# google-research/rigl

Measured on NVIDIA H100. Metric: sparse_train_step_images_per_sec_resnet50_erk80, higher is better.
Workload: dtype bf16

## Files before the change

include/rigl_b200.h:

```cpp
#ifndef RIGL_B200_H_
#define RIGL_B200_H_

#include <stddef.h>
#include <stdint.h>

#if defined(__GNUC__)
#define RIGL_API __attribute__((visibility("default")))
#else
#define RIGL_API
#endif

#ifdef __cplusplus
extern "C" {
#endif

typedef enum {
  RIGL_OK = 0,
  RIGL_ERR_INVALID_ARG = -1,
  RIGL_ERR_CUDA = -2,
  RIGL_ERR_WORKSPACE = -3,
  RIGL_ERR_UNSUPPORTED = -4,
  RIGL_ERR_DRIVER = -5
} rigl_status;

RIGL_API int rigl_version(void);
RIGL_API const char* rigl_last_error(void);
RIGL_API uint64_t rigl_launch_count(void);

RIGL_API int64_t rigl_mask_words(int64_t n);
RIGL_API int rigl_mask_pack_f32(const float* src, int64_t n, uint32_t* bits, void* stream);
RIGL_API int rigl_mask_unpack_f32(const uint32_t* bits, int64_t n, float* dst, void* stream);
RIGL_API int rigl_mask_popcount(const uint32_t* bits, int64_t n, int32_t* out_count_dev, void* stream);
RIGL_API int rigl_apply_mask_f32(const float* src, const uint32_t* bits, int64_t n, float* dst,
                        float scale, void* stream);

typedef struct {
  float* weights;
  const float* score_grow;
  uint32_t* mask_bits;
  const float* noise;
  float* slots[2];
  const float* grow_values;
  const float* score_drop;
  int64_t n;
  int32_t n_prune_override;
  int32_t flags;
  uint32_t noise_key;
  uint32_t reserved;
  const float* grad;
} rigl_layer_desc;

#define RIGL_LAYER_GROW_SCORE_SIGNED 1
#define RIGL_LAYER_DROP_ONLY 2
#define RIGL_LAYER_ALL_ACTIVE 4

typedef enum {
  RIGL_GROW_ZEROS = 0,
  RIGL_GROW_TENSOR = 1,
  RIGL_GROW_GRAD_SCALE = 2,
  RIGL_GROW_GRAD_SIGN = 3
} rigl_grow_mode;

typedef struct rigl_mask_plan rigl_mask_plan;

RIGL_API int rigl_mask_plan_create(const rigl_layer_desc* layers, int n_layers, rigl_mask_plan** out);
RIGL_API int rigl_mask_plan_destroy(rigl_mask_plan* plan);
RIGL_API size_t rigl_mask_plan_workspace_bytes(const rigl_mask_plan* plan);
RIGL_API int rigl_mask_update_run(rigl_mask_plan* plan, float drop_fraction, int grow_mode,
                         float grow_divisor, float acc_scale, int reinit_when_same,
                         void* workspace, size_t workspace_bytes, void* stream);
RIGL_API int rigl_mask_update_run_noise(rigl_mask_plan* plan, float drop_fraction, int grow_mode,
                         float grow_divisor, float acc_scale, int reinit_when_same, float noise_std,
                         uint64_t noise_seed, void* workspace, size_t workspace_bytes, void* stream);
RIGL_API int rigl_mask_noise_fill(float* out, int64_t n, uint32_t layer_noise_key, float noise_std,
                         uint64_t noise_seed, void* stream);
RIGL_API int rigl_mask_plan_read_stats(const rigl_mask_plan* plan, const void* workspace,
                              int32_t* out_host, void* stream);

RIGL_API size_t rigl_packed_weights_bytes(int taps, int cin, int cout);
RIGL_API int rigl_pack_masked_weights(const float* w_hwio, const uint32_t* mask_bits, int taps,
                                      int cin, int cout, void* packed, void* stream);

typedef struct {
  const float* weights;
  const uint32_t* mask_bits;
  void* packed;
  int32_t taps, cin, cout, reserved;
} rigl_pack_desc;
typedef struct rigl_pack_plan rigl_pack_plan;
RIGL_API int rigl_pack_plan_create(const rigl_pack_desc* layers, int n_layers, rigl_pack_plan** out);
RIGL_API int rigl_pack_plan_destroy(rigl_pack_plan* plan);
RIGL_API int rigl_pack_plan_run(rigl_pack_plan* plan, void* stream);

typedef struct {
  float* param;
  float* momentum;
  const float* grad;
  const uint32_t* mask_bits;
  int64_t n;
  float weight_decay;
  float grad_scale;
} rigl_sgd_desc;
typedef struct rigl_sgd_plan rigl_sgd_plan;
RIGL_API int rigl_sgd_plan_create(const rigl_sgd_desc* params, int n_params, rigl_sgd_plan** out);
RIGL_API int rigl_sgd_plan_destroy(rigl_sgd_plan* plan);
RIGL_API int rigl_sgd_plan_run(rigl_sgd_plan* plan, const float* lr_dev, float momentum, int nesterov, void* stream);

typedef struct {
  float* param;
  float* m;
  float* v;
  const float* grad;
  const uint32_t* mask_bits;
  int64_t n;
  float weight_decay;
  float grad_scale;
} rigl_adam_desc;
typedef struct rigl_adam_plan rigl_adam_plan;
RIGL_API int rigl_adam_plan_create(const rigl_adam_desc* params, int n_params, rigl_adam_plan** out);
RIGL_API int rigl_adam_plan_destroy(rigl_adam_plan* plan);
RIGL_API int rigl_adam_plan_run(rigl_adam_plan* plan, const float* lr_dev, float* powers_dev, float beta1, float beta2,
                                float epsilon, void* stream);

typedef struct {
  int32_t batch, in_h, in_w, cin;
  int32_t out_h, out_w, cout;
  int32_t ksize, stride, pad;
  int32_t x_pitch;
} rigl_conv_desc;

RIGL_API size_t rigl_conv_workspace_bytes(const rigl_conv_desc* d);
RIGL_API int rigl_masked_conv2d_fprop(const rigl_conv_desc* d, const void* x, const void* packed,
                                      void* y_bf16, float* y_f32, const float* bias, void* ws,
                                      size_t ws_bytes, void* stream);
RIGL_API int rigl_bn_partial_rows(void);
RIGL_API int rigl_masked_conv2d_fprop_bnstats(const rigl_conv_desc* d, const void* x, const void* packed,
                                              void* y_bf16, float* bn_partial, int* bn_rows_out, void* ws,
                                              size_t ws_bytes, void* stream);
RIGL_API int rigl_set_bn_stats_always(int on);
RIGL_API int rigl_masked_conv2d_fprop_bnapply(const rigl_conv_desc* d, const void* x, const void* packed,
                                              const void* residual, const float* scale, const float* shift, int relu,
                                              void* y_bf16, void* ws, size_t ws_bytes, void* stream);
RIGL_API int rigl_masked_conv2d_dgrad(const rigl_conv_desc* d, const void* dy, const void* packed,
                                      void* dx, void* ws, size_t ws_bytes, void* stream);
RIGL_API int rigl_conv2d_wgrad_dense(const rigl_conv_desc* d, const void* x, const void* dy,
                                     float* dw, float beta, void* ws, size_t ws_bytes, void* stream);
RIGL_API int rigl_im2col_nhwc(const rigl_conv_desc* d, const void* x, void* out, int64_t out_pitch,
                              void* stream);
RIGL_API int rigl_stem_s2d_supported(const rigl_conv_desc* d);
RIGL_API size_t rigl_stem_s2d_folded_bytes(const rigl_conv_desc* d);
RIGL_API size_t rigl_stem_s2d_packed_bytes(const rigl_conv_desc* d);
RIGL_API size_t rigl_stem_s2d_workspace_bytes(const rigl_conv_desc* d);
RIGL_API int rigl_stem_s2d_fold_input(const rigl_conv_desc* d, const void* x, void* xs, void* stream);
RIGL_API int rigl_stem_s2d_pack_weights(const rigl_conv_desc* d, const float* w_hwio,
                                        const uint32_t* mask_bits, void* packed, void* stream);
RIGL_API int rigl_stem_s2d_fprop(const rigl_conv_desc* d, const void* xs, const void* packed, void* y,
                                 void* stream);
RIGL_API int rigl_stem_s2d_wgrad(const rigl_conv_desc* d, const void* xs, const void* dy, float* dw,
                                 float beta, void* ws, size_t ws_bytes, void* stream);

RIGL_API size_t rigl_bn_workspace_bytes(int64_t rows, int channels);
RIGL_API int rigl_bn_forward_train(const void* y, const void* residual, const float* gamma,
                                   const float* beta, int64_t rows, int channels, float eps,
                                   float momentum, int relu, float* running_mean, float* running_var,
                                   float* save_mean, float* save_rstd, float* save_scale,
                                   float* save_shift, void* out, void* ws, size_t ws_bytes, void* relu_bits,
                                   void* stream);
RIGL_API int rigl_bn_forward_train_partials(const void* y, const void* residual, const float* gamma,
                                            const float* beta, const float* partial, int partial_rows,
                                            int64_t rows, int channels, float eps, float momentum, int relu,
                                            float* running_mean, float* running_var, float* save_mean,
                                            float* save_rstd, float* save_scale, float* save_shift, void* out,
                                            void* relu_bits, void* stream);
RIGL_API int rigl_bn_apply(const void* y, const void* residual, const float* scale, const float* shift,
                           int64_t rows, int channels, int relu, void* out, void* stream);
RIGL_API int rigl_bn_backward(const void* da, const void* da2, const void* y, const float* save_mean,
                              const float* save_rstd, const float* save_scale, const float* save_shift,
                              int64_t rows, int channels, int relu, void* dy, void* dresidual, float* dgamma,
                              float* dbeta, void* ws, size_t ws_bytes, const void* relu_bits, void* stream);

RIGL_API int rigl_maxpool_same_forward(const void* x, int n, int h, int w, int c, int ksize, int stride,
                                       void* y, uint8_t* argmax, void* stream);
RIGL_API int rigl_maxpool_same_backward(const void* dy, const uint8_t* argmax, int n, int h, int w, int c,
                                        int ksize, int stride, void* dx, void* stream);

RIGL_API size_t rigl_depthwise3x3_workspace_bytes(int n, int h, int w, int c, int stride);
RIGL_API int rigl_depthwise3x3_fprop(const void* x, const float* weights, int n, int h, int w, int c, int stride,
                                     void* y, void* stream);
RIGL_API int rigl_depthwise3x3_dgrad(const void* dy, const float* weights, int n, int h, int w, int c, int stride,
                                     void* dx, void* stream);
RIGL_API int rigl_depthwise3x3_wgrad(const void* x, const void* dy, int n, int h, int w, int c, int stride,
                                     float* dw, float beta, void* ws, size_t ws_bytes, void* stream);

RIGL_API int rigl_set_force_simt(int on);

#ifdef __cplusplus
}
#endif
#endif
```

rigl_b200/_cabi.py:

```python
import ctypes as C
import os

_HERE = os.path.dirname(os.path.abspath(__file__))
LIB_PATH = os.path.join(_HERE, 'librigl_b200.so')
_lib = None
ABI_VERSION = 202


class RiglError(RuntimeError):
  pass


class LayerDesc(C.Structure):
  _fields_ = [('weights', C.c_void_p), ('score_grow', C.c_void_p), ('mask_bits', C.c_void_p),
              ('noise', C.c_void_p), ('slots', C.c_void_p * 2), ('grow_values', C.c_void_p), ('score_drop', C.c_void_p),
              ('n', C.c_int64), ('n_prune_override', C.c_int32), ('flags', C.c_int32), ('noise_key', C.c_uint32),
              ('reserved', C.c_uint32), ('grad', C.c_void_p)]


class PackDesc(C.Structure):
  _fields_ = [('weights', C.c_void_p), ('mask_bits', C.c_void_p), ('packed', C.c_void_p),
              ('taps', C.c_int32), ('cin', C.c_int32), ('cout', C.c_int32), ('reserved', C.c_int32)]


class SgdDesc(C.Structure):
  _fields_ = [('param', C.c_void_p), ('momentum', C.c_void_p), ('grad', C.c_void_p), ('mask_bits', C.c_void_p),
              ('n', C.c_int64), ('weight_decay', C.c_float), ('grad_scale', C.c_float)]


class AdamDesc(C.Structure):
  _fields_ = [('param', C.c_void_p), ('m', C.c_void_p), ('v', C.c_void_p), ('grad', C.c_void_p),
              ('mask_bits', C.c_void_p), ('n', C.c_int64), ('weight_decay', C.c_float), ('grad_scale', C.c_float)]


class ConvDesc(C.Structure):
  _fields_ = [('batch', C.c_int32), ('in_h', C.c_int32), ('in_w', C.c_int32), ('cin', C.c_int32),
              ('out_h', C.c_int32), ('out_w', C.c_int32), ('cout', C.c_int32),
              ('ksize', C.c_int32), ('stride', C.c_int32), ('pad', C.c_int32), ('x_pitch', C.c_int32)]


GROW_ZEROS, GROW_TENSOR, GROW_GRAD_SCALE, GROW_GRAD_SIGN = 0, 1, 2, 3
LAYER_GROW_SCORE_SIGNED, LAYER_DROP_ONLY, LAYER_ALL_ACTIVE = 1, 2, 4

_vp, _i64, _i32, _f32, _sz = C.c_void_p, C.c_int64, C.c_int, C.c_float, C.c_size_t

SIGNATURES = {
    'rigl_version': (C.c_int, []),
    'rigl_last_error': (C.c_char_p, []),
    'rigl_launch_count': (C.c_uint64, []),
    'rigl_mask_words': (_i64, [_i64]),
    'rigl_mask_pack_f32': (C.c_int, [_vp, _i64, _vp, _vp]),
    'rigl_mask_unpack_f32': (C.c_int, [_vp, _i64, _vp, _vp]),
    'rigl_mask_popcount': (C.c_int, [_vp, _i64, _vp, _vp]),
    'rigl_apply_mask_f32': (C.c_int, [_vp, _vp, _i64, _vp, _f32, _vp]),
    'rigl_mask_plan_create': (C.c_int, [C.POINTER(LayerDesc), _i32, C.POINTER(_vp)]),
    'rigl_mask_plan_destroy': (C.c_int, [_vp]),
    'rigl_mask_plan_workspace_bytes': (_sz, [_vp]),
    'rigl_mask_update_run': (C.c_int, [_vp, _f32, _i32, _f32, _f32, _i32, _vp, _sz, _vp]),
    'rigl_mask_update_run_noise': (C.c_int, [_vp, _f32, _i32, _f32, _f32, _i32, _f32, C.c_uint64, _vp, _sz, _vp]),
    'rigl_mask_noise_fill': (C.c_int, [_vp, _i64, C.c_uint32, _f32, C.c_uint64, _vp]),
    'rigl_mask_plan_read_stats': (C.c_int, [_vp, _vp, C.POINTER(C.c_int32), _vp]),
    'rigl_packed_weights_bytes': (_sz, [_i32, _i32, _i32]),
    'rigl_pack_masked_weights': (C.c_int, [_vp, _vp, _i32, _i32, _i32, _vp, _vp]),
    'rigl_pack_plan_create': (C.c_int, [C.POINTER(PackDesc), _i32, C.POINTER(_vp)]),
    'rigl_pack_plan_destroy': (C.c_int, [_vp]),
    'rigl_pack_plan_run': (C.c_int, [_vp, _vp]),
    'rigl_sgd_plan_create': (C.c_int, [C.POINTER(SgdDesc), _i32, C.POINTER(_vp)]),
    'rigl_sgd_plan_destroy': (C.c_int, [_vp]),
    'rigl_sgd_plan_run': (C.c_int, [_vp, _vp, _f32, _i32, _vp]),
    'rigl_adam_plan_create': (C.c_int, [C.POINTER(AdamDesc), _i32, C.POINTER(_vp)]),
    'rigl_adam_plan_destroy': (C.c_int, [_vp]),
    'rigl_adam_plan_run': (C.c_int, [_vp, _vp, _vp, _f32, _f32, _f32, _vp]),
    'rigl_conv_workspace_bytes': (_sz, [C.POINTER(ConvDesc)]),
    'rigl_masked_conv2d_fprop': (C.c_int, [C.POINTER(ConvDesc), _vp, _vp, _vp, _vp, _vp, _vp, _sz, _vp]),
    'rigl_bn_partial_rows': (C.c_int, []),
    'rigl_set_bn_stats_always': (C.c_int, [_i32]),
    'rigl_masked_conv2d_fprop_bnstats': (C.c_int, [C.POINTER(ConvDesc), _vp, _vp, _vp, _vp, C.POINTER(C.c_int), _vp, _sz, _vp]),
    'rigl_masked_conv2d_fprop_bnapply': (C.c_int, [C.POINTER(ConvDesc), _vp, _vp, _vp, _vp, _vp, _i32, _vp, _vp, _sz,
                                                   _vp]),
    'rigl_masked_conv2d_dgrad': (C.c_int, [C.POINTER(ConvDesc), _vp, _vp, _vp, _vp, _sz, _vp]),
    'rigl_conv2d_wgrad_dense': (C.c_int, [C.POINTER(ConvDesc), _vp, _vp, _vp, _f32, _vp, _sz, _vp]),
    'rigl_im2col_nhwc': (C.c_int, [C.POINTER(ConvDesc), _vp, _vp, _i64, _vp]),
    'rigl_stem_s2d_supported': (C.c_int, [C.POINTER(ConvDesc)]),
    'rigl_stem_s2d_folded_bytes': (_sz, [C.POINTER(ConvDesc)]),
    'rigl_stem_s2d_packed_bytes': (_sz, [C.POINTER(ConvDesc)]),
    'rigl_stem_s2d_workspace_bytes': (_sz, [C.POINTER(ConvDesc)]),
    'rigl_stem_s2d_fold_input': (C.c_int, [C.POINTER(ConvDesc), _vp, _vp, _vp]),
    'rigl_stem_s2d_pack_weights': (C.c_int, [C.POINTER(ConvDesc), _vp, _vp, _vp, _vp]),
    'rigl_stem_s2d_fprop': (C.c_int, [C.POINTER(ConvDesc), _vp, _vp, _vp, _vp]),
    'rigl_stem_s2d_wgrad': (C.c_int, [C.POINTER(ConvDesc), _vp, _vp, _vp, _f32, _vp, _sz, _vp]),
    'rigl_bn_workspace_bytes': (_sz, [_i64, _i32]),
    'rigl_bn_forward_train': (C.c_int, [_vp, _vp, _vp, _vp, _i64, _i32, _f32, _f32, _i32, _vp, _vp, _vp, _vp,
                                        _vp, _vp, _vp, _vp, _sz, _vp, _vp]),
    'rigl_bn_forward_train_partials': (C.c_int, [_vp, _vp, _vp, _vp, _vp, _i32, _i64, _i32, _f32, _f32, _i32, _vp, _vp,
                                                 _vp, _vp, _vp, _vp, _vp, _vp, _vp]),
    'rigl_bn_apply': (C.c_int, [_vp, _vp, _vp, _vp, _i64, _i32, _i32, _vp, _vp]),
    'rigl_bn_backward': (C.c_int, [_vp, _vp, _vp, _vp, _vp, _vp, _vp, _i64, _i32, _i32, _vp, _vp, _vp, _vp,
                                   _vp, _sz, _vp, _vp]),
    'rigl_depthwise3x3_workspace_bytes': (_sz, [_i32, _i32, _i32, _i32, _i32]),
    'rigl_depthwise3x3_fprop': (C.c_int, [_vp, _vp, _i32, _i32, _i32, _i32, _i32, _vp, _vp]),
    'rigl_depthwise3x3_dgrad': (C.c_int, [_vp, _vp, _i32, _i32, _i32, _i32, _i32, _vp, _vp]),
    'rigl_depthwise3x3_wgrad': (C.c_int, [_vp, _vp, _i32, _i32, _i32, _i32, _i32, _vp, _f32, _vp, _sz, _vp]),
    'rigl_maxpool_same_forward': (C.c_int, [_vp, _i32, _i32, _i32, _i32, _i32, _i32, _vp, _vp, _vp]),
    'rigl_maxpool_same_backward': (C.c_int, [_vp, _vp, _i32, _i32, _i32, _i32, _i32, _i32, _vp, _vp]),
    'rigl_set_force_simt': (C.c_int, [_i32]),
}


def lib():
  global _lib
  if _lib is None:
    if not os.path.exists(LIB_PATH):
      raise RiglError('librigl_b200.so not built: run `python -m rigl_b200.build` '
                      '(or __graft_entry__.build()); there is no CPU fallback')
    handle = C.CDLL(LIB_PATH)
    for name, (res, args) in SIGNATURES.items():
      fn = getattr(handle, name)
      fn.restype = res
      fn.argtypes = args
    if handle.rigl_version() < ABI_VERSION:
      raise RiglError('librigl_b200.so is older (rigl_version %d) than this package needs (%d): rebuild with '
                      '`python -m rigl_b200.build`' % (handle.rigl_version(), ABI_VERSION))
    _lib = handle
  return _lib


def check(status, what=''):
  if status != 0:
    msg = lib().rigl_last_error().decode('utf-8', 'replace')
    raise RiglError('%s failed (%d): %s' % (what or 'rigl call', status, msg))


def stream_ptr():
  import torch
  return torch.cuda.current_stream().cuda_stream


def launch_count():
  return int(lib().rigl_launch_count())
```

rigl_b200/csrc/conv_api.cu:

```cuda
#include <stdlib.h>

#include "common.cuh"
#include "conv_common.cuh"

namespace rigl {

static int g_force_simt = -1;

static bool force_simt() {
  if (g_force_simt < 0) {
    const char* e = getenv("RIGL_FORCE_SIMT");
    g_force_simt = (e && e[0] == '1') ? 1 : 0;
  }
  return g_force_simt == 1;
}

int geom_from_desc(const rigl_conv_desc* d, ConvGeom* g) {
  RIGL_REQUIRE(d != nullptr, "null conv desc");
  RIGL_REQUIRE(d->batch > 0 && d->in_h > 0 && d->in_w > 0 && d->cin > 0 && d->cout > 0 && d->ksize > 0 &&
                   d->stride > 0 && d->pad >= 0,
               "conv desc: non-positive dimension");
  RIGL_REQUIRE(d->pad < d->ksize && d->out_h > 0 && d->out_w > 0 &&
                   (d->out_h - 1) * d->stride - d->pad < d->in_h && (d->out_w - 1) * d->stride - d->pad < d->in_w,
               "conv desc: output %dx%d inconsistent with input %dx%d, k=%d, stride=%d, pad=%d", d->out_h,
               d->out_w, d->in_h, d->in_w, d->ksize, d->stride, d->pad);
  g->batch = d->batch; g->in_h = d->in_h; g->in_w = d->in_w; g->cin = d->cin;
  g->out_h = d->out_h; g->out_w = d->out_w; g->cout = d->cout;
  g->ksize = d->ksize; g->stride = d->stride; g->pad = d->pad;
  g->cin_pad = round_up8(d->cin); g->cout_pad = round_up8(d->cout);
  g->x_pitch = d->x_pitch > 0 ? d->x_pitch : d->cin;
  RIGL_REQUIRE(g->x_pitch >= d->cin, "conv desc: x_pitch %d < cin %d", g->x_pitch, d->cin);
  return RIGL_OK;
}

}

using namespace rigl;

extern "C" int rigl_im2col_nhwc(const rigl_conv_desc* d, const void* x, void* out, int64_t out_pitch,
                                void* stream) {
  ConvGeom g;
  int rc = geom_from_desc(d, &g);
  if (rc != RIGL_OK) return rc;
  RIGL_REQUIRE(x && out && out_pitch >= (int64_t)g.taps() * g.cin, "rigl_im2col_nhwc: bad arguments");
  return simt_im2col(g, x, out, out_pitch, (cudaStream_t)stream);
}

extern "C" int rigl_stem_s2d_supported(const rigl_conv_desc* d) {
  ConvGeom g;
  if (geom_from_desc(d, &g) != RIGL_OK) return 0;
  return s2d_supported(g) && !force_simt() ? 1 : 0;
}
extern "C" size_t rigl_stem_s2d_folded_bytes(const rigl_conv_desc* d) {
  ConvGeom g;
  return geom_from_desc(d, &g) == RIGL_OK ? s2d_folded_bytes(g) : 0;
}
extern "C" size_t rigl_stem_s2d_packed_bytes(const rigl_conv_desc* d) {
  ConvGeom g;
  return geom_from_desc(d, &g) == RIGL_OK ? s2d_packed_bytes(g) : 0;
}
extern "C" size_t rigl_stem_s2d_workspace_bytes(const rigl_conv_desc* d) {
  ConvGeom g;
  return geom_from_desc(d, &g) == RIGL_OK ? s2d_workspace_bytes(g) : 0;
}
extern "C" int rigl_stem_s2d_fold_input(const rigl_conv_desc* d, const void* x, void* xs, void* stream) {
  ConvGeom g;
  int rc = geom_from_desc(d, &g);
  if (rc != RIGL_OK) return rc;
  RIGL_REQUIRE(x && xs && s2d_supported(g) && aligned16(xs), "rigl_stem_s2d_fold_input: bad arguments");
  return s2d_fold(g, x, xs, (cudaStream_t)stream);
}
extern "C" int rigl_stem_s2d_pack_weights(const rigl_conv_desc* d, const float* w_hwio, const uint32_t* mask_bits,
                                          void* packed, void* stream) {
  ConvGeom g;
  int rc = geom_from_desc(d, &g);
  if (rc != RIGL_OK) return rc;
  RIGL_REQUIRE(w_hwio && mask_bits && packed && s2d_supported(g), "rigl_stem_s2d_pack_weights: bad arguments");
  return s2d_pack(g, w_hwio, mask_bits, packed, (cudaStream_t)stream);
}
extern "C" int rigl_stem_s2d_fprop(const rigl_conv_desc* d, const void* xs, const void* packed, void* y,
                                   void* stream) {
  ConvGeom g;
  int rc = geom_from_desc(d, &g);
  if (rc != RIGL_OK) return rc;
  RIGL_REQUIRE(xs && packed && y && s2d_supported(g), "rigl_stem_s2d_fprop: bad arguments");
  return s2d_fprop(g, xs, packed, y, (cudaStream_t)stream);
}
extern "C" int rigl_stem_s2d_wgrad(const rigl_conv_desc* d, const void* xs, const void* dy, float* dw, float beta,
                                   void* ws, size_t ws_bytes, void* stream) {
  ConvGeom g;
  int rc = geom_from_desc(d, &g);
  if (rc != RIGL_OK) return rc;
  RIGL_REQUIRE(xs && dy && dw && s2d_supported(g), "rigl_stem_s2d_wgrad: bad arguments");
  return s2d_wgrad(g, xs, dy, dw, beta, ws, ws_bytes, (cudaStream_t)stream);
}

extern "C" int rigl_set_force_simt(int on) {
  g_force_simt = on ? 1 : 0;
  return RIGL_OK;
}

extern "C" size_t rigl_conv_workspace_bytes(const rigl_conv_desc* d) {
  ConvGeom g;
  if (geom_from_desc(d, &g) != RIGL_OK) return 0;
  return tc_workspace_bytes(g);
}

extern "C" int rigl_masked_conv2d_fprop(const rigl_conv_desc* d, const void* x, const void* packed,
                                        void* y_bf16, float* y_f32, const float* bias, void* ws,
                                        size_t ws_bytes, void* stream) {
  ConvGeom g;
  int rc = geom_from_desc(d, &g);
  if (rc != RIGL_OK) return rc;
  RIGL_REQUIRE(x && packed && (y_bf16 || y_f32), "rigl_masked_conv2d_fprop: null tensor");
  const PackedLayout L = packed_layout(g.taps(), g.cin, g.cout);
  if (!force_simt() && tc_supported(g, 0))
    return tc_fprop(g, x, packed, y_bf16, y_f32, bias, ws, ws_bytes, (cudaStream_t)stream);
  return simt_fprop(g, x, static_cast<const uint8_t*>(packed) + L.off_dgrad, y_bf16, y_f32, bias,
                    (cudaStream_t)stream);
}

extern "C" int rigl_bn_partial_rows(void) { return tc_max_ctas(); }

extern "C" int rigl_set_bn_stats_always(int on) {
  tc_set_bn_stats_always(on != 0);
  return RIGL_OK;
}

extern "C" int rigl_masked_conv2d_fprop_bnstats(const rigl_conv_desc* d, const void* x, const void* packed,
                                                void* y_bf16, float* bn_partial, int* bn_rows_out, void* ws,
                                                size_t ws_bytes, void* stream) {
  ConvGeom g;
  int rc = geom_from_desc(d, &g);
  if (rc != RIGL_OK) return rc;
  RIGL_REQUIRE(x && packed && y_bf16 && bn_partial && bn_rows_out, "rigl_masked_conv2d_fprop_bnstats: null argument");
  if (force_simt() || !tc_supported(g, 0)) {
    set_error("rigl_masked_conv2d_fprop_bnstats: shape not on the tensor-core path");
    return RIGL_ERR_UNSUPPORTED;
  }
  return tc_fprop(g, x, packed, y_bf16, nullptr, nullptr, ws, ws_bytes, (cudaStream_t)stream, bn_partial, bn_rows_out);
}

extern "C" int rigl_masked_conv2d_fprop_bnapply(const rigl_conv_desc* d, const void* x, const void* packed,
                                                const void* residual, const float* scale, const float* shift, int relu,
                                                void* y_bf16, void* ws, size_t ws_bytes, void* stream) {
  ConvGeom g;
  int rc = geom_from_desc(d, &g);
  if (rc != RIGL_OK) return rc;
  RIGL_REQUIRE(x && packed && scale && shift && y_bf16, "rigl_masked_conv2d_fprop_bnapply: null argument");
  RIGL_REQUIRE(g.cout % 8 == 0, "rigl_masked_conv2d_fprop_bnapply: cout %d is not a multiple of 8", g.cout);
  RIGL_REQUIRE(aligned16(x) && aligned16(y_bf16) && aligned16(residual),
               "rigl_masked_conv2d_fprop_bnapply: tensors must be 16-byte aligned");
  if (force_simt() || !tc_supported(g, 0)) {
    set_error("rigl_masked_conv2d_fprop_bnapply: shape not on the K-major tensor-core kernel");
    return RIGL_ERR_UNSUPPORTED;
  }
  const BnApplyArgs bn = {residual, scale, shift, relu};
  return tc_fprop(g, x, packed, y_bf16, nullptr, nullptr, ws, ws_bytes, (cudaStream_t)stream, nullptr, nullptr, &bn);
}

extern "C" int rigl_masked_conv2d_dgrad(const rigl_conv_desc* d, const void* dy, const void* packed,
                                        void* dx, void* ws, size_t ws_bytes, void* stream) {
  ConvGeom g;
  int rc = geom_from_desc(d, &g);
  if (rc != RIGL_OK) return rc;
  RIGL_REQUIRE(dy && packed && dx, "rigl_masked_conv2d_dgrad: null tensor");
  const PackedLayout L = packed_layout(g.taps(), g.cin, g.cout);
  if (!force_simt() && tc_supported(g, 1))
    return tc_dgrad(g, dy, packed, dx, ws, ws_bytes, (cudaStream_t)stream);
  return simt_dgrad(g, dy, static_cast<const uint8_t*>(packed) + L.off_fprop, dx, (cudaStream_t)stream);
}

extern "C" int rigl_conv2d_wgrad_dense(const rigl_conv_desc* d, const void* x, const void* dy, float* dw,
                                       float beta, void* ws, size_t ws_bytes, void* stream) {
  ConvGeom g;
  int rc = geom_from_desc(d, &g);
  if (rc != RIGL_OK) return rc;
  RIGL_REQUIRE(x && dy && dw, "rigl_conv2d_wgrad_dense: null tensor");
  RIGL_REQUIRE(beta == 0.f || beta == 1.f, "rigl_conv2d_wgrad_dense: beta must be 0 or 1");
  if (!force_simt() && tc_supported(g, 2))
    return tc_wgrad(g, x, dy, dw, beta, ws, ws_bytes, (cudaStream_t)stream);
  return simt_wgrad(g, x, dy, dw, beta, (cudaStream_t)stream);
}
```

rigl_b200/csrc/conv_common.cuh:

```cuda
#pragma once
#include <stdint.h>
#include <stddef.h>

#include "../../include/rigl_b200.h"

namespace rigl {

struct ConvGeom {
  int batch, in_h, in_w, cin;
  int out_h, out_w, cout;
  int ksize, stride, pad;
  int cin_pad, cout_pad;
  int x_pitch;
  __host__ __device__ int64_t out_pixels() const { return (int64_t)batch * out_h * out_w; }
  __host__ __device__ int64_t in_pixels() const { return (int64_t)batch * in_h * in_w; }
  __host__ __device__ int taps() const { return ksize * ksize; }
};

inline int round_up8(int v) { return (v + 7) / 8 * 8; }

struct PackedLayout {
  size_t off_fprop, off_dgrad, off_nnz, total;
  int cin_pad, cout_pad, n_tiles, k_tiles;
};

inline PackedLayout packed_layout(int taps, int cin, int cout) {
  PackedLayout L;
  L.cin_pad = round_up8(cin);
  L.cout_pad = round_up8(cout);
  L.n_tiles = (cout + 63) / 64;
  L.k_tiles = (cin + 63) / 64;
  auto up = [](size_t v) { return (v + 255) / 256 * 256; };
  L.off_fprop = 0;
  L.off_dgrad = up((size_t)taps * cout * L.cin_pad * 2);
  L.off_nnz = L.off_dgrad + up((size_t)taps * cin * L.cout_pad * 2);
  L.total = L.off_nnz + up((size_t)taps * L.n_tiles * L.k_tiles * 4);
  return L;
}

int geom_from_desc(const rigl_conv_desc* d, ConvGeom* g);

int simt_fprop(const ConvGeom& g, const void* x, const void* w_dgrad, void* y, float* y_f32,
               const float* bias, cudaStream_t s);
int simt_dgrad(const ConvGeom& g, const void* dy, const void* w_fprop, void* dx, cudaStream_t s);
int simt_wgrad(const ConvGeom& g, const void* x, const void* dy, float* dw, float beta, cudaStream_t s);
int simt_im2col(const ConvGeom& g, const void* x, void* out, int64_t out_pitch, cudaStream_t s);

struct BnApplyArgs {
  const void* residual;
  const float* scale;
  const float* shift;
  int relu;
};

bool tc_supported(const ConvGeom& g, int which );
size_t tc_workspace_bytes(const ConvGeom& g);
int tc_fprop(const ConvGeom& g, const void* x, const void* packed, void* y, float* y_f32,
             const float* bias, void* ws, size_t ws_bytes, cudaStream_t s, float* bn_partial = nullptr,
             int* bn_rows = nullptr, const BnApplyArgs* bn_apply = nullptr);
int tc_max_ctas();
void tc_set_bn_stats_always(bool on);
int tc_dgrad(const ConvGeom& g, const void* dy, const void* packed, void* dx, void* ws,
             size_t ws_bytes, cudaStream_t s);
int tc_wgrad(const ConvGeom& g, const void* x, const void* dy, float* dw, float beta, void* ws,
             size_t ws_bytes, cudaStream_t s);

bool s2d_supported(const ConvGeom& g);
size_t s2d_folded_bytes(const ConvGeom& g);
size_t s2d_packed_bytes(const ConvGeom& g);
size_t s2d_workspace_bytes(const ConvGeom& g);
int s2d_fold(const ConvGeom& g, const void* x, void* xs, cudaStream_t s);
int s2d_pack(const ConvGeom& g, const float* w, const uint32_t* bits, void* packed, cudaStream_t s);
int s2d_fprop(const ConvGeom& g, const void* xs, const void* packed, void* y, cudaStream_t s);
int s2d_wgrad(const ConvGeom& g, const void* xs, const void* dy, float* dw, float beta, void* ws, size_t ws_bytes,
              cudaStream_t s);

}
```

rigl_b200/csrc/igemm_tc.cu:

```cuda
#include <cuda.h>
#include <cuda_bf16.h>

#include <stdio.h>
#include <stdlib.h>

#include <mutex>

#include "common.cuh"
#include "conv_common.cuh"
#include "tc_ptx.cuh"

namespace rigl {

using namespace ptx;

constexpr int kMaxTaps = 9;
constexpr int kBM = 128;
constexpr int kBK = 64;
constexpr int kThreads = 384;
constexpr int kConsumerWarp0 = 4;
constexpr int kConsumerWarps = 8;
constexpr int kConsumerThreads = 256;

struct TapInfo {
  int8_t map_id, dh, dw, pad;
  int32_t b_tap;
};

struct IgemmParams {
  int ntaps;
  TapInfo taps[kMaxTaps];
  int kblks;
  int GW, GH, NB;
  int bw, bh, bn;
  int tiles_w, tiles_h, tiles_n;
  int n_tiles;
  int N;
  __nv_bfloat16* out_bf16;
  float* out_f32;
  const float* bias;
  long long o_off, o_sn, o_sh, o_sw;
  const uint32_t* nnz;
  int nnz_tap_stride, nnz_n_stride, nnz_k_stride;
  int tma_store;
  float* bn_partial;
};

struct BnEpilogue {
  const float* scale;
  const float* shift;
  int relu;
  int residual;
};

struct TMaps4 {
  CUtensorMap a[4];
};

__device__ __forceinline__ bool weight_block_live(const IgemmParams& p, int tap_idx, int n_tile, int kb, int bn64) {
  if (p.nnz == nullptr) return true;
  const uint32_t* base = p.nnz + (long long)p.taps[tap_idx].b_tap * p.nnz_tap_stride + (long long)kb * p.nnz_k_stride;
  uint32_t s = 0;
  for (int j = 0; j < bn64; ++j) {
    const int nt = n_tile * bn64 + j;
    if ((long long)nt * 64 < p.N) s += __ldg(base + (long long)nt * p.nnz_n_stride);
  }
  return s != 0;
}


constexpr int kLiveWords = 10;
__device__ __forceinline__ bool live_mask_used(const IgemmParams& p) {
  return p.nnz != nullptr && p.ntaps * p.kblks <= kLiveWords * 32;
}
template <int kBN64>
__device__ __forceinline__ bool build_live_mask(const IgemmParams& p, int n_tile, int lane, uint32_t* mask_smem) {
  const int nkb = p.ntaps * p.kblks;
  if (!live_mask_used(p)) return false;
  for (int w = 0; w * 32 < nkb; ++w) {
    const int j = w * 32 + lane;
    bool live = true;
    if (j > 0 && j < nkb) live = weight_block_live(p, j / p.kblks, n_tile, j % p.kblks, kBN64);
    const uint32_t m = __ballot_sync(0xffffffffu, live);
    if (lane == 0) mask_smem[w] = m;
  }
  __syncwarp();
  return true;
}

__device__ __forceinline__ void slab_bn_stats(uint32_t slab, int quad, int lane, float* __restrict__ bn_row, int co0,
                                              int n) {
  const int cp = lane & 7, g = lane >> 3;
  const uint32_t chunk = (uint32_t)(2 * quad + (cp >> 2));
  const uint32_t word = (uint32_t)(cp & 3) * 4u;
  float s0 = 0.f, s1 = 0.f, q0 = 0.f, q1 = 0.f;
#pragma unroll 8
  for (int i = 0; i < 32; ++i) {
    const uint32_t row = (uint32_t)(32 * g + ((i + 2 * g) & 31));
    uint32_t v;
    asm volatile("ld.shared.b32 %0, [%1];" : "=r"(v) : "r"(slab + row * 128u + (((chunk ^ (row & 7u)) << 4) | word)));
    const float a = __uint_as_float(v << 16), b = __uint_as_float(v & 0xffff0000u);
    s0 += a; s1 += b;
    q0 = fmaf(a, a, q0); q1 = fmaf(b, b, q1);
  }
#pragma unroll
  for (int o = 8; o <= 16; o <<= 1) {
    s0 += __shfl_xor_sync(0xffffffffu, s0, o); s1 += __shfl_xor_sync(0xffffffffu, s1, o);
    q0 += __shfl_xor_sync(0xffffffffu, q0, o); q1 += __shfl_xor_sync(0xffffffffu, q1, o);
  }
  const int co = co0 + 16 * quad + 2 * cp;
  if (g == 0 && co < n) {
    atomicAdd(bn_row + co, s0); atomicAdd(bn_row + co + 1, s1);
    atomicAdd(bn_row + n + co, q0); atomicAdd(bn_row + n + co + 1, q1);
  }
}

template <int S, int R>
__device__ __forceinline__ void stage_slab(const float (&d)[R], uint32_t slab, int row, bool ok0, bool ok1, int lane) {
#pragma unroll
  for (int jj = 0; jj < 8; ++jj) {
#pragma unroll
    for (int h = 0; h < 2; ++h) {
      const int r = row + 8 * h;
      const int e = 4 * (8 * S + jj) + 2 * h;
      __nv_bfloat162 v = __floats2bfloat162_rn(d[e], d[e + 1]);
      const uint32_t w = (h ? ok1 : ok0) ? *reinterpret_cast<uint32_t*>(&v) : 0u;
      const uint32_t dst = slab + (uint32_t)r * 128u + (uint32_t)((jj ^ (r & 7)) << 4) + (uint32_t)(lane & 3) * 4u;
      asm volatile("st.shared.b32 [%0], %1;" ::"r"(dst), "r"(w) : "memory");
    }
  }
}

template <int S, int R>
__device__ __forceinline__ void stage_slab_bn(const float (&d)[R], uint32_t slab, int row, bool ok0, bool ok1, int lane,
                                              const BnEpilogue& ep, int co0, int n) {
#pragma unroll
  for (int jj = 0; jj < 8; ++jj) {
    const int co = co0 + 8 * jj + 2 * (lane & 3);
    float sc0 = 0.f, sc1 = 0.f, sh0 = 0.f, sh1 = 0.f;
    if (co < n) {
      sc0 = __ldg(ep.scale + co); sc1 = __ldg(ep.scale + co + 1);
      sh0 = __ldg(ep.shift + co); sh1 = __ldg(ep.shift + co + 1);
    }
#pragma unroll
    for (int h = 0; h < 2; ++h) {
      const int r = row + 8 * h;
      const int e = 4 * (8 * S + jj) + 2 * h;
      const uint32_t dst = slab + (uint32_t)r * 128u + (uint32_t)((jj ^ (r & 7)) << 4) + (uint32_t)(lane & 3) * 4u;
      const float2 f = __bfloat1622float2(__floats2bfloat162_rn(d[e], d[e + 1]));
      float a = fmaf(f.x, sc0, sh0), b = fmaf(f.y, sc1, sh1);
      if (ep.residual) {
        uint32_t rw;
        asm volatile("ld.shared.b32 %0, [%1];" : "=r"(rw) : "r"(dst) : "memory");
        a += __uint_as_float(rw << 16);
        b += __uint_as_float(rw & 0xffff0000u);
      }
      if (ep.relu) { a = fmaxf(a, 0.f); b = fmaxf(b, 0.f); }
      __nv_bfloat162 v = __floats2bfloat162_rn(a, b);
      const uint32_t w = (h ? ok1 : ok0) ? *reinterpret_cast<uint32_t*>(&v) : 0u;
      asm volatile("st.shared.b32 [%0], %1;" ::"r"(dst), "r"(w) : "memory");
    }
  }
}

template <int R>
__device__ __forceinline__ void zero_acc(float (&d)[R]) {
#pragma unroll
  for (int i = 0; i < R; ++i) d[i] = 0.f;
}

template <int CL>
__device__ __forceinline__ void release_stage(uint32_t bar) {
  if (CL == 1) {
    mbar_arrive(bar);
  } else {
#pragma unroll
    for (int c = 0; c < CL; ++c) mbar_arrive_cluster(bar, (uint32_t)c);
  }
}

template <int BN, int STAGES, int CL, bool kBnApply>
__device__ __forceinline__ void kmajor_body(const TMaps4& amaps, const CUtensorMap& bmap, const CUtensorMap& omap,
                                            const IgemmParams& p, const CUtensorMap* rmap, const BnEpilogue& ep) {
  extern __shared__ __align__(1024) uint8_t smem_raw[];
  constexpr uint32_t kABytes = kBM * kBK * 2;
  constexpr uint32_t kBBytes = BN * kBK * 2;
  constexpr uint32_t kStageBytes = kABytes + kBBytes;
  constexpr uint32_t kSlabBytes = kBM * 64 * 2;
  const uint32_t smem_base = (smem_u32(smem_raw) + 1023u) & ~1023u;
  const uint32_t out_base = smem_base + STAGES * kStageBytes;
  const uint32_t bar_base = out_base + 2 * kSlabBytes;
  auto full_bar = [&](int s) { return bar_base + 8u * s; };
  auto empty_bar = [&](int s) { return bar_base + 8u * (STAGES + s); };
  const uint32_t res_bar = bar_base + 8u * (2 * STAGES);

  __shared__ uint32_t live_prod[kLiveWords], live_cons[2][2][kLiveWords];
  const int warp = threadIdx.x >> 5, lane = threadIdx.x & 31;
  if (threadIdx.x == 0) {
    for (int i = 0; i < 4; ++i) prefetch_tmap(&amaps.a[i]);
    prefetch_tmap(&bmap);
    if (p.tma_store) prefetch_tmap(&omap);
    for (int s = 0; s < STAGES; ++s) { mbar_init(full_bar(s), 1); mbar_init(empty_bar(s), kConsumerWarps * CL); }
    if constexpr (kBnApply) {
      mbar_init(res_bar, 1);
      if (ep.residual) prefetch_tmap(rmap);
    }
    fence_barrier_init();
  }
  if (CL > 1) cluster_sync_all(); else __syncthreads();

  const uint32_t cta_rank = CL > 1 ? cluster_ctarank() : 0u;
  const int m_tiles = p.tiles_w * p.tiles_h * p.tiles_n;
  const int total = (m_tiles + CL - 1) / CL * p.n_tiles;
  const int cluster_id = blockIdx.x / CL, n_clusters = gridDim.x / CL;
  constexpr int kBN64 = (BN + 63) / 64;
  constexpr uint16_t kMcMask = (uint16_t)((1u << CL) - 1u);

  if (warp == 0) {
    int stage = 0; uint32_t phase = 0;
    for (int tile = cluster_id; tile < total; tile += n_clusters) {
      const int n_tile = tile % p.n_tiles;
      const int m_tile = (tile / p.n_tiles) * CL + (int)cta_rank;
      const int tw = m_tile % p.tiles_w;
      const int th = (m_tile / p.tiles_w) % p.tiles_h;
      const int tn = m_tile / (p.tiles_w * p.tiles_h);
      const bool masked = build_live_mask<kBN64>(p, n_tile, lane, live_prod);
      int j = 0;
      for (int t = 0; t < p.ntaps; ++t) {
        const TapInfo tap = p.taps[t];
        for (int kb = 0; kb < p.kblks; ++kb, ++j) {
          if (masked && !((live_prod[j >> 5] >> (j & 31)) & 1u)) continue;
          if (CL > 1) mbar_wait_cluster(empty_bar(stage), phase ^ 1u);
          else mbar_wait(empty_bar(stage), phase ^ 1u);
          if (elect_one()) {
            const uint32_t a_dst = smem_base + stage * kStageBytes;
            mbar_arrive_expect_tx(full_bar(stage), kStageBytes);
            tma_load_4d(a_dst, &amaps.a[tap.map_id], full_bar(stage), kb * kBK, tw * p.bw + tap.dw,
                        th * p.bh + tap.dh, tn * p.bn);
            if (CL > 1)
              tma_load_3d_mc(a_dst + kABytes + cta_rank * (uint32_t)(BN / CL) * 128u, &bmap, full_bar(stage),
                             kb * kBK, n_tile * BN + (int)cta_rank * (BN / CL), tap.b_tap, kMcMask);
            else
              tma_load_3d(a_dst + kABytes, &bmap, full_bar(stage), kb * kBK, n_tile * BN, tap.b_tap);
          }
          __syncwarp();
          if (++stage == STAGES) { stage = 0; phase ^= 1u; }
        }
      }
    }
  } else if (warp >= kConsumerWarp0) {
    const int cw = warp - kConsumerWarp0;
    const int wg = cw >> 2;
    const int row = 64 * wg + 16 * (cw & 3) + (lane >> 2);
    const bool issuer = (cw == 0 && lane == 0);
    float acc[BN / 2];
    int stage = 0; uint32_t phase = 0;
    uint32_t slab_ctr = 0;
    uint32_t res_phase = 0;
    float* bn_row = (!kBnApply && p.bn_partial) ? p.bn_partial + (size_t)blockIdx.x * 2 * p.N : nullptr;
    if (bn_row) {
      for (int i = cw * 32 + lane; i < 2 * p.N; i += kConsumerThreads) bn_row[i] = 0.f;
      __threadfence_block();
      named_bar_sync(1, kConsumerThreads);
    }
    int tile_ctr = 0;
    for (int tile = cluster_id; tile < total; tile += n_clusters, ++tile_ctr) {
      const int n_tile = tile % p.n_tiles;
      const int m_tile = (tile / p.n_tiles) * CL + (int)cta_rank;
      uint32_t* live = live_cons[wg][tile_ctr & 1];
      if ((cw & 3) == 0) build_live_mask<kBN64>(p, n_tile, lane, live);
      named_bar_sync(3 + wg, 128);
      const bool masked = live_mask_used(p);
      zero_acc(acc);
      int prev = -1;
      const int nkb = p.ntaps * p.kblks;
      for (int j = 0; j < nkb; ++j) {
        if (masked && !((live[j >> 5] >> (j & 31)) & 1u)) continue;
        mbar_wait(full_bar(stage), phase);
        const uint32_t a_src = smem_base + stage * kStageBytes;
        const uint64_t da = make_smem_desc(a_src + (uint32_t)wg * 64u * 128u, 16, 1024);
        const uint64_t db = make_smem_desc(a_src + kABytes, 16, 1024);
        fence_regs(acc);
        wgmma_fence();
#pragma unroll
        for (int k = 0; k < kBK / 16; ++k)
          Wgmma<BN>::template ss<0, 0>(acc, da + 2 * k, db + 2 * k);
        wgmma_commit();
        wgmma_wait<1>();
        if (prev >= 0 && lane == 0) release_stage<CL>(empty_bar(prev));
        prev = stage;
        if (++stage == STAGES) { stage = 0; phase ^= 1u; }
      }
      wgmma_wait<0>();
      fence_regs(acc);
      if (prev >= 0 && lane == 0) release_stage<CL>(empty_bar(prev));

      const int tw = m_tile % p.tiles_w;
      const int th = (m_tile / p.tiles_w) % p.tiles_h;
      const int tn = m_tile / (p.tiles_w * p.tiles_h);
      bool ok[2]; long long o_pix[2];
#pragma unroll
      for (int h = 0; h < 2; ++h) {
        const int r = row + 8 * h;
        const int pw = tw * p.bw + r % p.bw;
        const int ph = th * p.bh + (r / p.bw) % p.bh;
        const int pn = tn * p.bn + r / (p.bw * p.bh);
        ok[h] = pw < p.GW && ph < p.GH && pn < p.NB;
        o_pix[h] = p.o_off + pn * p.o_sn + ph * p.o_sh + pw * p.o_sw;
      }
      if (kBnApply || p.tma_store) {
#pragma unroll
        for (int s = 0; s < kBN64; ++s) {
          const int co0 = n_tile * BN + 64 * s;
          if (co0 >= p.N) break;
          const uint32_t slab = out_base + (uint32_t)(slab_ctr & 1) * kSlabBytes;
          if (issuer) tma_store_wait_read<1>();
          named_bar_sync(1, kConsumerThreads);
          if constexpr (kBnApply) {
            if (ep.residual) {
              if (issuer) {
                mbar_arrive_expect_tx(res_bar, kSlabBytes);
                tma_load_4d(slab, rmap, res_bar, co0, tw * p.bw, th * p.bh, tn * p.bn);
              }
              mbar_wait(res_bar, res_phase);
              res_phase ^= 1u;
            }
            if (s == 0) stage_slab_bn<0>(acc, slab, row, ok[0], ok[1], lane, ep, co0, p.N);
            else stage_slab_bn<(kBN64 > 1 ? 1 : 0)>(acc, slab, row, ok[0], ok[1], lane, ep, co0, p.N);
          } else {
            if (s == 0) stage_slab<0>(acc, slab, row, ok[0], ok[1], lane);
            else stage_slab<(kBN64 > 1 ? 1 : 0)>(acc, slab, row, ok[0], ok[1], lane);
          }
          fence_proxy_async_smem();
          named_bar_sync(1, kConsumerThreads);
          if (issuer) {
            tma_store_4d(&omap, slab, co0, tw * p.bw, th * p.bh, tn * p.bn);
            tma_store_commit();
          }
          if (bn_row && wg == 0) slab_bn_stats(slab, cw, lane, bn_row, co0, p.N);
          ++slab_ctr;
        }
      } else {
#pragma unroll
        for (int jc = 0; jc < BN / 8; ++jc) {
#pragma unroll
          for (int h = 0; h < 2; ++h) {
#pragma unroll
            for (int e = 0; e < 2; ++e) {
              const int co = n_tile * BN + 8 * jc + 2 * (lane & 3) + e;
              if (ok[h] && co < p.N) {
                float a = acc[4 * jc + 2 * h + e];
                if (p.bias) a += __ldg(p.bias + co);
                if (p.out_bf16) p.out_bf16[o_pix[h] + co] = __float2bfloat16(a);
                if (p.out_f32) p.out_f32[o_pix[h] + co] = a;
              }
            }
          }
        }
      }
    }
    if (p.tma_store && issuer) tma_store_wait_all();
  }
  if (CL > 1) cluster_sync_all();
}

template <int BN, int STAGES, int CL>
__global__ void __launch_bounds__(kThreads, 1)
k_igemm_kmajor(const __grid_constant__ TMaps4 amaps, const __grid_constant__ CUtensorMap bmap,
               const __grid_constant__ CUtensorMap omap, const IgemmParams p) {
  kmajor_body<BN, STAGES, CL, false>(amaps, bmap, omap, p, nullptr, BnEpilogue{});
}

template <int BN, int STAGES, int CL>
__global__ void __launch_bounds__(kThreads, 1)
k_igemm_kmajor_bn(const __grid_constant__ TMaps4 amaps, const __grid_constant__ CUtensorMap bmap,
                  const __grid_constant__ CUtensorMap omap, const IgemmParams p,
                  const __grid_constant__ CUtensorMap rmap, const BnEpilogue ep) {
  kmajor_body<BN, STAGES, CL, true>(amaps, bmap, omap, p, &rmap, ep);
}

struct WgradParams {
  int ntaps;
  TapInfo taps[kMaxTaps];
  int GW, GH, NB;
  int bw, bh, bn;
  int tiles_w, tiles_h, tiles_n;
  int pblocks, splits, pblocks_per_split;
  int ci, co;
  int m_tiles, n_tiles;
  float* out;
  long long split_stride;
};

template <int BN, int STAGES, int CL>
__global__ void __launch_bounds__(kThreads, 1)
k_igemm_wgrad(const __grid_constant__ TMaps4 xmaps, const __grid_constant__ CUtensorMap dymap,
              const WgradParams p) {
  extern __shared__ __align__(1024) uint8_t smem_raw[];
  constexpr uint32_t kABytes = kBM * kBK * 2;
  constexpr uint32_t kBBytes = BN * kBK * 2;
  constexpr uint32_t kStageBytes = kABytes + kBBytes;
  constexpr uint32_t kBox = 64 * 64 * 2;
  constexpr int kBBoxes = BN / 64;
  static_assert(CL == 1 || kBBoxes % CL == 0, "multicast splits the dY boxes between the CTAs");
  constexpr uint16_t kMcMask = (uint16_t)((1u << CL) - 1u);

  const uint32_t smem_base = (smem_u32(smem_raw) + 1023u) & ~1023u;
  const uint32_t bar_base = smem_base + STAGES * kStageBytes;
  auto full_bar = [&](int s) { return bar_base + 8u * s; };
  auto empty_bar = [&](int s) { return bar_base + 8u * (STAGES + s); };

  const int warp = threadIdx.x >> 5, lane = threadIdx.x & 31;
  if (threadIdx.x == 0) {
    for (int i = 0; i < 4; ++i) prefetch_tmap(&xmaps.a[i]);
    prefetch_tmap(&dymap);
    for (int s = 0; s < STAGES; ++s) { mbar_init(full_bar(s), 1); mbar_init(empty_bar(s), kConsumerWarps * CL); }
    fence_barrier_init();
  }
  if (CL > 1) cluster_sync_all(); else __syncthreads();

  const uint32_t cta_rank = CL > 1 ? cluster_ctarank() : 0u;
  const int mcount = p.ntaps * p.m_tiles;
  const int m_groups = (mcount + CL - 1) / CL;
  const int groups_per_split = m_groups * p.n_tiles;
  const int total_groups = groups_per_split * p.splits;
  const int cluster_id = blockIdx.x / CL, n_clusters = gridDim.x / CL;

  if (warp == 0) {
    int stage = 0; uint32_t phase = 0;
    for (int q = cluster_id; q < total_groups; q += n_clusters) {
      const int split = q / groups_per_split;
      const int r = q % groups_per_split;
      const int n_tile = r % p.n_tiles;
      const int mi = (r / p.n_tiles) * CL + (int)cta_rank;
      const bool live = mi < mcount;
      const TapInfo tap = p.taps[live ? mi / p.m_tiles : 0];
      const int c_base = live ? (mi % p.m_tiles) * kBM : (1 << 28);
      const int pb0 = split * p.pblocks_per_split;
      const int pb1 = min(pb0 + p.pblocks_per_split, p.pblocks);
      int tw = pb0 % p.tiles_w, th = (pb0 / p.tiles_w) % p.tiles_h, tn = pb0 / (p.tiles_w * p.tiles_h);
      for (int pb = pb0; pb < pb1; ++pb) {
        if (CL > 1) mbar_wait_cluster(empty_bar(stage), phase ^ 1u);
        else mbar_wait(empty_bar(stage), phase ^ 1u);
        if (elect_one()) {
          const uint32_t a_dst = smem_base + stage * kStageBytes;
          const uint32_t b_dst = a_dst + kABytes;
          mbar_arrive_expect_tx(full_bar(stage), kStageBytes);
#pragma unroll
          for (int h = 0; h < kBM / 64; ++h)
            tma_load_4d(a_dst + h * kBox, &xmaps.a[tap.map_id], full_bar(stage), c_base + h * 64,
                        tw * p.bw + tap.dw, th * p.bh + tap.dh, tn * p.bn);
          if (CL > 1) {
#pragma unroll
            for (int hh = 0; hh < kBBoxes / CL; ++hh) {
              const int h = (int)cta_rank * (kBBoxes / CL) + hh;
              tma_load_4d_mc(b_dst + h * kBox, &dymap, full_bar(stage), n_tile * BN + h * 64, tw * p.bw,
                             th * p.bh, tn * p.bn, kMcMask);
            }
          } else {
#pragma unroll
            for (int h = 0; h < kBBoxes; ++h)
              tma_load_4d(b_dst + h * kBox, &dymap, full_bar(stage), n_tile * BN + h * 64, tw * p.bw,
                          th * p.bh, tn * p.bn);
          }
        }
        __syncwarp();
        if (++tw == p.tiles_w) { tw = 0; if (++th == p.tiles_h) { th = 0; ++tn; } }
        if (++stage == STAGES) { stage = 0; phase ^= 1u; }
      }
    }
  } else if (warp >= kConsumerWarp0) {
    const int cw = warp - kConsumerWarp0;
    const int wg = cw >> 2;
    const int row = 64 * wg + 16 * (cw & 3) + (lane >> 2);
    float acc[BN / 2];
    int stage = 0; uint32_t phase = 0;
    for (int q = cluster_id; q < total_groups; q += n_clusters) {
      const int split = q / groups_per_split;
      const int r = q % groups_per_split;
      const int n_tile = r % p.n_tiles;
      const int mi = (r / p.n_tiles) * CL + (int)cta_rank;
      const bool live = mi < mcount;
      const int tap_idx = live ? mi / p.m_tiles : 0;
      const int pb0 = split * p.pblocks_per_split;
      const int pb1 = min(pb0 + p.pblocks_per_split, p.pblocks);
      zero_acc(acc);
      int prev = -1;
      for (int pb = pb0; pb < pb1; ++pb) {
        mbar_wait(full_bar(stage), phase);
        const uint32_t a_src = smem_base + stage * kStageBytes;
        const uint64_t da = make_smem_desc(a_src + (uint32_t)wg * kBox, kBox, 1024);
        const uint64_t db = make_smem_desc(a_src + kABytes, kBox, 1024);
        fence_regs(acc);
        wgmma_fence();
#pragma unroll
        for (int k = 0; k < kBK / 16; ++k)
          Wgmma<BN>::template ss<1, 1>(acc, da + 128 * k, db + 128 * k);
        wgmma_commit();
        wgmma_wait<1>();
        if (prev >= 0 && lane == 0) release_stage<CL>(empty_bar(prev));
        prev = stage;
        if (++stage == STAGES) { stage = 0; phase ^= 1u; }
      }
      wgmma_wait<0>();
      fence_regs(acc);
      if (prev >= 0 && lane == 0) release_stage<CL>(empty_bar(prev));

      const int m0 = live ? (mi % p.m_tiles) * kBM : p.ci;
      float* base = p.out + (long long)split * p.split_stride + (long long)p.taps[tap_idx].b_tap * p.ci * p.co;
#pragma unroll
      for (int h = 0; h < 2; ++h) {
        const int ci = m0 + row + 8 * h;
        if (ci >= p.ci) continue;
#pragma unroll
        for (int jc = 0; jc < BN / 8; ++jc) {
          const int co = n_tile * BN + 8 * jc + 2 * (lane & 3);
          if (co < p.co)
            *reinterpret_cast<float2*>(base + (long long)ci * p.co + co) =
                make_float2(acc[4 * jc + 2 * h], acc[4 * jc + 2 * h + 1]);
        }
      }
    }
  }
  if (CL > 1) cluster_sync_all();
}

__global__ void k_splitk_reduce(const float* __restrict__ part, long long split_stride, int splits,
                                float* __restrict__ dw, long long n, float beta) {
  const long long i = ((long long)blockIdx.x * blockDim.x + threadIdx.x) * 4;
  if (i >= n) return;
  if (i + 3 < n) {
    float4 acc = beta != 0.f ? *reinterpret_cast<const float4*>(dw + i) : make_float4(0.f, 0.f, 0.f, 0.f);
    for (int s = 0; s < splits; ++s) {
      const float4 v = *reinterpret_cast<const float4*>(part + (long long)s * split_stride + i);
      acc.x += v.x; acc.y += v.y; acc.z += v.z; acc.w += v.w;
    }
    *reinterpret_cast<float4*>(dw + i) = acc;
  } else {
    for (long long j = i; j < n; ++j) {
      float a = beta != 0.f ? dw[j] : 0.f;
      for (int s = 0; s < splits; ++s) a += part[(long long)s * split_stride + j];
      dw[j] = a;
    }
  }
}

typedef CUresult (*EncodeTiledFn)(CUtensorMap*, CUtensorMapDataType, cuuint32_t, void*, const cuuint64_t*,
                                  const cuuint64_t*, const cuuint32_t*, const cuuint32_t*, CUtensorMapInterleave,
                                  CUtensorMapSwizzle, CUtensorMapL2promotion, CUtensorMapFloatOOBfill);

static EncodeTiledFn g_encode = nullptr;
static bool g_tma_store = true;
static bool g_cluster_mc = false;
static bool g_bn_stats_always = false;
static bool g_halo = true;
static int g_num_sms = 0;
static std::once_flag g_once;
static int g_init_status = RIGL_OK;

static void init_driver() {
  void* fn = nullptr;
  cudaDriverEntryPointQueryResult qres;
  cudaError_t e = cudaGetDriverEntryPoint("cuTensorMapEncodeTiled", &fn, cudaEnableDefault, &qres);
  if (e != cudaSuccess || fn == nullptr || qres != cudaDriverEntryPointSuccess) {
    set_error("cuTensorMapEncodeTiled not available from the driver (%s)", cudaGetErrorString(e));
    g_init_status = RIGL_ERR_DRIVER;
    return;
  }
  g_encode = reinterpret_cast<EncodeTiledFn>(fn);
  if (const char* e = getenv("RIGL_TMA_STORE")) g_tma_store = !(e[0] == '0');
  if (const char* e = getenv("RIGL_HALO3X3")) g_halo = !(e[0] == '0');
  if (const char* e = getenv("RIGL_CLUSTER_MC")) g_cluster_mc = (e[0] == '1');
  int dev = 0;
  cudaGetDevice(&dev);
  cudaDeviceGetAttribute(&g_num_sms, cudaDevAttrMultiProcessorCount, dev);
  if (g_num_sms <= 0) g_num_sms = kNumSmsHint;
}

static int ensure_driver() {
  static thread_local bool ctx_ready = false;
  if (!ctx_ready) {
    cudaFree(0);
    ctx_ready = true;
  }
  std::call_once(g_once, init_driver);
  return g_init_status;
}

static int make_tmap_swz(CUtensorMap* out, const void* base, int rank, const uint64_t* dims,
                         const uint64_t* strides_bytes , const uint32_t* box, CUtensorMapSwizzle swz) {
  cuuint32_t estr[5] = {1, 1, 1, 1, 1};
  cuuint64_t gdim[5], gstr[4];
  cuuint32_t bx[5];
  for (int i = 0; i < rank; ++i) { gdim[i] = dims[i]; bx[i] = box[i]; }
  for (int i = 0; i + 1 < rank; ++i) gstr[i] = strides_bytes[i];
  CUresult r = g_encode(out, CU_TENSOR_MAP_DATA_TYPE_BFLOAT16, (cuuint32_t)rank, const_cast<void*>(base), gdim,
                        gstr, bx, estr, CU_TENSOR_MAP_INTERLEAVE_NONE, swz,
                        CU_TENSOR_MAP_L2_PROMOTION_L2_128B, CU_TENSOR_MAP_FLOAT_OOB_FILL_NONE);
  if (r != CUDA_SUCCESS) {
    set_error("cuTensorMapEncodeTiled failed (%d): rank %d dims [%llu,%llu,%llu,%llu] box [%u,%u,%u,%u]", (int)r,
              rank, (unsigned long long)dims[0], (unsigned long long)(rank > 1 ? dims[1] : 0),
              (unsigned long long)(rank > 2 ? dims[2] : 0), (unsigned long long)(rank > 3 ? dims[3] : 0), box[0],
              rank > 1 ? box[1] : 0, rank > 2 ? box[2] : 0, rank > 3 ? box[3] : 0);
    return RIGL_ERR_DRIVER;
  }
  return RIGL_OK;
}
static int make_tmap(CUtensorMap* out, const void* base, int rank, const uint64_t* dims,
                     const uint64_t* strides_bytes , const uint32_t* box) {
  return make_tmap_swz(out, base, rank, dims, strides_bytes, box, CU_TENSOR_MAP_SWIZZLE_128B);
}

static int make_act_map(CUtensorMap* out, const void* base, int nb, int h, int w, int c, int pitch, int s, int rh,
                        int rw, const uint32_t box[4]) {
  const uint64_t hr = (h - rh + s - 1) / s, wr = (w - rw + s - 1) / s;
  const uint64_t dims[4] = {(uint64_t)c, wr, hr, (uint64_t)nb};
  const uint64_t strides[3] = {(uint64_t)s * pitch * 2, (uint64_t)s * w * pitch * 2, (uint64_t)h * w * pitch * 2};
  const uint8_t* p = static_cast<const uint8_t*>(base) + ((size_t)rh * w + rw) * pitch * 2;
  return make_tmap(out, p, 4, dims, strides, box);
}

static void choose_box(int gw, int gh, int nb, int total, int* bw, int* bh, int* bn) {
  long long best = -1;
  for (int w = 1; w <= total; w *= 2)
    for (int h = 1; w * h <= total; h *= 2) {
      const int n = total / (w * h);
      const long long padded = (long long)((gw + w - 1) / w * w) * ((gh + h - 1) / h * h) * ((nb + n - 1) / n * n);
      const long long score = padded * 1024 - w * 16 - h;
      if (best < 0 || score < best) { best = score; *bw = w; *bh = h; *bn = n; }
    }
}

static inline int floordiv(int a, int b) { return (a >= 0) ? a / b : -((-a + b - 1) / b); }
static inline int posmod(int a, int b) { return ((a % b) + b) % b; }

template <typename P>
static void set_pixel_tiling(P& p, int gw, int gh, int nb, int box_pixels) {
  p.GW = gw; p.GH = gh; p.NB = nb;
  choose_box(gw, gh, nb, box_pixels, &p.bw, &p.bh, &p.bn);
  p.tiles_w = (gw + p.bw - 1) / p.bw; p.tiles_h = (gh + p.bh - 1) / p.bh; p.tiles_n = (nb + p.bn - 1) / p.bn;
}

template <typename P>
static int set_conv_taps(P& p, TMaps4* maps, const ConvGeom& g, const void* x, const uint32_t box[4]) {
  bool made[4] = {false, false, false, false};
  p.ntaps = 0;
  for (int kh = 0; kh < g.ksize; ++kh)
    for (int kw = 0; kw < g.ksize; ++kw) {
      const int rh = posmod(kh - g.pad, g.stride), rw = posmod(kw - g.pad, g.stride);
      const int id = rh * g.stride + rw;
      if (!made[id]) {
        const int rc = make_act_map(&maps->a[id], x, g.batch, g.in_h, g.in_w, g.cin, g.x_pitch, g.stride, rh, rw, box);
        if (rc != RIGL_OK) return rc;
        made[id] = true;
      }
      TapInfo& t = p.taps[p.ntaps++];
      t.map_id = (int8_t)id; t.dh = (int8_t)floordiv(kh - g.pad, g.stride); t.dw = (int8_t)floordiv(kw - g.pad, g.stride);
      t.b_tap = kh * g.ksize + kw;
    }
  for (int i = 0; i < 4; ++i) if (!made[i]) maps->a[i] = maps->a[p.taps[0].map_id];
  return RIGL_OK;
}

int tc_max_ctas() {
  ensure_driver();
  return g_num_sms > 0 ? g_num_sms : kNumSmsHint;
}

bool tc_supported(const ConvGeom& g, int which) {
  if (g.x_pitch % 8 || g.cout % 8) return false;
  if (which == 1 && g.cin % 8) return false;
  if (g.stride != 1 && g.stride != 2) return false;
  if (g.ksize * g.ksize > kMaxTaps) return false;
  (void)which;
  return true;
}

static size_t wgrad_ws_elems(const ConvGeom& g, int* splits_out, int* bps_out, int bw, int bh, int bn, int bn_tile) {
  const int tiles_w = (g.out_w + bw - 1) / bw, tiles_h = (g.out_h + bh - 1) / bh, tiles_n = (g.batch + bn - 1) / bn;
  const int pblocks = tiles_w * tiles_h * tiles_n;
  const int out_tiles = g.taps() * ((g.cin + kBM - 1) / kBM) * ((g.cout + bn_tile - 1) / bn_tile);
  const int sms = g_num_sms > 0 ? g_num_sms : kNumSmsHint;
  int splits = (2 * sms + out_tiles - 1) / out_tiles;
  if (splits > pblocks) splits = pblocks;
  if (splits < 1) splits = 1;
  const int bps = (pblocks + splits - 1) / splits;
  splits = (pblocks + bps - 1) / bps;
  if (splits_out) *splits_out = splits;
  if (bps_out) *bps_out = bps;
  return (size_t)splits * g.taps() * g.cin * g.cout;
}

static int wgrad_bn_tile(const ConvGeom& g) { return g.cout >= 128 ? 128 : 64; }

#include "halo3x3.cuh"
#include "stem_s2d.cuh"

size_t tc_workspace_bytes(const ConvGeom& g) {
  if (!tc_supported(g, 2)) return 0;
  int bw, bh, bn;
  choose_box(g.out_w, g.out_h, g.batch, 64, &bw, &bh, &bn);
  size_t elems = wgrad_ws_elems(g, nullptr, nullptr, bw, bh, bn, wgrad_bn_tile(g));
  HaloParams hp;
  if (halo_wgrad_ok(g, &hp)) { const size_t e = halo_wgrad_ws_elems(g, hp); if (e > elems) elems = e; }
  return elems * sizeof(float) + 256;
}

static bool kmajor_use_mc(const IgemmParams& p) {
  return g_cluster_mc && p.tiles_w * p.tiles_h * p.tiles_n >= 2;
}
static int kmajor_b_rows(const IgemmParams& p, int bn_tile) {
  return kmajor_use_mc(p) ? bn_tile / 2 : bn_tile;
}

static int kmajor_grid(const IgemmParams& p) {
  const int cl = kmajor_use_mc(p) ? 2 : 1;
  const int m_tiles = p.tiles_w * p.tiles_h * p.tiles_n;
  const int pairs = ((m_tiles + cl - 1) / cl) * p.n_tiles;
  int clusters = g_num_sms / cl;
  if (pairs < clusters) clusters = pairs;
  return clusters * cl;
}

template <int CL, typename Kern, typename... Args>
static int launch_clustered(Kern kern, int grid, size_t smem, cudaStream_t s, Args... args) {
  if (CL == 1) {
    kern<<<(unsigned)grid, kThreads, smem, s>>>(args...);
    return RIGL_OK;
  }
  cudaLaunchConfig_t cfg = {};
  cfg.gridDim = dim3((unsigned)grid);
  cfg.blockDim = dim3(kThreads);
  cfg.dynamicSmemBytes = smem;
  cfg.stream = s;
  cudaLaunchAttribute attr[1];
  attr[0].id = cudaLaunchAttributeClusterDimension;
  attr[0].val.clusterDim.x = CL; attr[0].val.clusterDim.y = 1; attr[0].val.clusterDim.z = 1;
  cfg.attrs = attr;
  cfg.numAttrs = 1;
  RIGL_CUDA(cudaLaunchKernelEx(&cfg, kern, args...));
  return RIGL_OK;
}

template <int BN, int STAGES, int CL>
static int launch_kmajor(const TMaps4& amaps, const CUtensorMap& bmap, const CUtensorMap& omap, const IgemmParams& p,
                         cudaStream_t s, const CUtensorMap* rmap, const BnEpilogue* ep) {
  constexpr size_t smem = (size_t)STAGES * (kBM * kBK * 2 + BN * kBK * 2) + 2 * (kBM * 64 * 2) + 1024 + 256;
  static_assert(smem <= 227 * 1024, "K-major kernel exceeds the shared memory of an SM");
  static_assert(8 * (2 * STAGES + 1) <= 256, "K-major kernel barriers exceed their shared memory");
  if (ep != nullptr) {
    static bool configured_bn = false;
    if (!configured_bn) {
      RIGL_CUDA(cudaFuncSetAttribute(k_igemm_kmajor_bn<BN, STAGES, CL>, cudaFuncAttributeMaxDynamicSharedMemorySize,
                                     (int)smem));
      configured_bn = true;
    }
    const int rc = launch_clustered<CL>(k_igemm_kmajor_bn<BN, STAGES, CL>, kmajor_grid(p), smem, s, amaps, bmap, omap,
                                        p, *rmap, *ep);
    if (rc != RIGL_OK) return rc;
    RIGL_LAUNCH_CHECK("k_igemm_kmajor_bn");
    return RIGL_OK;
  }
  static bool configured = false;
  if (!configured) {
    RIGL_CUDA(cudaFuncSetAttribute(k_igemm_kmajor<BN, STAGES, CL>, cudaFuncAttributeMaxDynamicSharedMemorySize, (int)smem));
    configured = true;
  }
  const int rc = launch_clustered<CL>(k_igemm_kmajor<BN, STAGES, CL>, kmajor_grid(p), smem, s, amaps, bmap, omap, p);
  if (rc != RIGL_OK) return rc;
  RIGL_LAUNCH_CHECK("k_igemm_kmajor");
  return RIGL_OK;
}

static int dispatch_kmajor(int n_out, const TMaps4& amaps, const CUtensorMap& bmap, const CUtensorMap& omap,
                           IgemmParams& p, int bn_tile, cudaStream_t s, const CUtensorMap* rmap = nullptr,
                           const BnEpilogue* ep = nullptr) {
  p.n_tiles = (n_out + bn_tile - 1) / bn_tile;
  const bool mc = kmajor_use_mc(p);
  if (bn_tile == 64)
    return mc ? launch_kmajor<64, 7, 2>(amaps, bmap, omap, p, s, rmap, ep)
              : launch_kmajor<64, 7, 1>(amaps, bmap, omap, p, s, rmap, ep);
  return mc ? launch_kmajor<128, 5, 2>(amaps, bmap, omap, p, s, rmap, ep)
            : launch_kmajor<128, 5, 1>(amaps, bmap, omap, p, s, rmap, ep);
}

static int pick_bn(int n_out) {
  return n_out > 64 ? 128 : 64;
}

void tc_set_bn_stats_always(bool on) { g_bn_stats_always = on; }

int tc_fprop(const ConvGeom& g, const void* x, const void* packed, void* y, float* y_f32, const float* bias,
             void* ws, size_t ws_bytes, cudaStream_t s, float* bn_partial, int* bn_rows, const BnApplyArgs* bn_apply) {
  (void)ws; (void)ws_bytes;
  int rc = ensure_driver();
  if (rc != RIGL_OK) return rc;
  const PackedLayout L = packed_layout(g.taps(), g.cin, g.cout);
  const uint8_t* pk = static_cast<const uint8_t*>(packed);
  {
    HaloParams hp = {};
    if (y != nullptr && y_f32 == nullptr && bias == nullptr && halo_fprop_ok(g, &hp)) {
      if (bn_apply != nullptr) {
        set_error("fused BN apply: layer runs on the halo kernels");
        return RIGL_ERR_UNSUPPORTED;
      }
      if (bn_partial != nullptr) {
        set_error("fused BN statistics: layer runs on the halo kernels");
        return RIGL_ERR_UNSUPPORTED;
      }
      return halo_launch_kmajor(hp, x, g.cin, g.x_pitch, pk + L.off_fprop, L.cin_pad, g.cout, y, g.cout, false, s);
    }
  }
  if (bn_partial != nullptr && !g_bn_stats_always) {
    const int K = g.taps() * g.cin;
    if (!(K >= 512 || (K >= 256 && g.cout <= 128))) {
      set_error("fused BN statistics: not profitable for this shape (K = %d, cout = %d)", K, g.cout);
      return RIGL_ERR_UNSUPPORTED;
    }
  }
  IgemmParams p = {};
  set_pixel_tiling(p, g.out_w, g.out_h, g.batch, 128);
  p.kblks = (g.cin + kBK - 1) / kBK;
  p.N = g.cout;
  p.out_bf16 = static_cast<__nv_bfloat16*>(y); p.out_f32 = y_f32; p.bias = bias;
  p.o_off = 0; p.o_sw = g.cout; p.o_sh = (long long)g.out_w * g.cout; p.o_sn = (long long)g.out_h * g.out_w * g.cout;
  p.nnz = reinterpret_cast<const uint32_t*>(pk + L.off_nnz);
  p.nnz_tap_stride = L.n_tiles * L.k_tiles; p.nnz_n_stride = L.k_tiles; p.nnz_k_stride = 1;
  p.bn_partial = bn_partial;
  TMaps4 amaps;
  const uint32_t abox[4] = {(uint32_t)kBK, (uint32_t)p.bw, (uint32_t)p.bh, (uint32_t)p.bn};
  rc = set_conv_taps(p, &amaps, g, x, abox);
  if (rc != RIGL_OK) return rc;
  const int bn_tile = pick_bn(g.cout);
  CUtensorMap bmap;
  const uint64_t bdims[3] = {(uint64_t)L.cin_pad, (uint64_t)g.cout, (uint64_t)g.taps()};
  const uint64_t bstr[2] = {(uint64_t)L.cin_pad * 2, (uint64_t)g.cout * L.cin_pad * 2};
  const uint32_t bbox[3] = {(uint32_t)kBK, (uint32_t)kmajor_b_rows(p, bn_tile), 1};
  rc = make_tmap(&bmap, pk + L.off_fprop, 3, bdims, bstr, bbox);
  if (rc != RIGL_OK) return rc;
  CUtensorMap omap = bmap;
  p.tma_store = (y != nullptr && y_f32 == nullptr && bias == nullptr && g_tma_store) ? 1 : 0;
  if (p.tma_store) {
    rc = make_act_map(&omap, y, g.batch, g.out_h, g.out_w, g.cout, g.cout, 1, 0, 0, abox);
    if (rc != RIGL_OK) return rc;
  }
  if (bn_partial) {
    if (!p.tma_store) {
      set_error("fused BN statistics need the bf16 TMA-store epilogue");
      return RIGL_ERR_UNSUPPORTED;
    }
    p.bn_partial = bn_partial;
    p.n_tiles = (g.cout + bn_tile - 1) / bn_tile;
    if (bn_rows) *bn_rows = kmajor_grid(p);
  }
  if (bn_apply) {
    if (!p.tma_store) {
      set_error("fused BN apply needs the bf16 TMA-store epilogue");
      return RIGL_ERR_UNSUPPORTED;
    }
    CUtensorMap rmap = omap;
    if (bn_apply->residual) {
      rc = make_act_map(&rmap, bn_apply->residual, g.batch, g.out_h, g.out_w, g.cout, g.cout, 1, 0, 0, abox);
      if (rc != RIGL_OK) return rc;
    }
    const BnEpilogue ep = {bn_apply->scale, bn_apply->shift, bn_apply->relu ? 1 : 0, bn_apply->residual ? 1 : 0};
    return dispatch_kmajor(g.cout, amaps, bmap, omap, p, bn_tile, s, &rmap, &ep);
  }
  return dispatch_kmajor(g.cout, amaps, bmap, omap, p, bn_tile, s);
}

int tc_dgrad(const ConvGeom& g, const void* dy, const void* packed, void* dx, void* ws, size_t ws_bytes,
             cudaStream_t s) {
  (void)ws; (void)ws_bytes;
  int rc = ensure_driver();
  if (rc != RIGL_OK) return rc;
  const PackedLayout L = packed_layout(g.taps(), g.cin, g.cout);
  const uint8_t* pk = static_cast<const uint8_t*>(packed);
  const int st = g.stride;
  {
    HaloParams hp = {};
    if (halo_dgrad_ok(g, &hp))
      return halo_launch_kmajor(hp, dy, g.cout, g.cout, pk + L.off_dgrad, L.cout_pad, g.cin, dx, g.x_pitch, true, s);
  }
  bool need_zero = false;
  for (int ph = 0; ph < st && !need_zero; ++ph)
    for (int pw = 0; pw < st; ++pw) {
      int n = 0;
      for (int kh = 0; kh < g.ksize; ++kh)
        for (int kw = 0; kw < g.ksize; ++kw)
          if (posmod(ph + g.pad - kh, st) == 0 && posmod(pw + g.pad - kw, st) == 0) ++n;
      if (n == 0) need_zero = true;
    }
  if (need_zero) RIGL_CUDA(cudaMemsetAsync(dx, 0, (size_t)g.in_pixels() * g.x_pitch * 2, s));
  for (int ph = 0; ph < st; ++ph)
    for (int pw = 0; pw < st; ++pw) {
      IgemmParams p = {};
      const int gh = (g.in_h - ph + st - 1) / st, gw = (g.in_w - pw + st - 1) / st;
      if (gh <= 0 || gw <= 0) continue;
      p.ntaps = 0;
      for (int kh = 0; kh < g.ksize; ++kh)
        for (int kw = 0; kw < g.ksize; ++kw)
          if (posmod(ph + g.pad - kh, st) == 0 && posmod(pw + g.pad - kw, st) == 0) {
            TapInfo& t = p.taps[p.ntaps++];
            t.map_id = 0; t.dh = (int8_t)((ph + g.pad - kh) / st); t.dw = (int8_t)((pw + g.pad - kw) / st);
            t.b_tap = kh * g.ksize + kw;
          }
      if (p.ntaps == 0) continue;
      set_pixel_tiling(p, gw, gh, g.batch, 128);
      p.kblks = (g.cout + kBK - 1) / kBK;
      p.N = g.cin;
      p.out_bf16 = static_cast<__nv_bfloat16*>(dx);
      p.o_off = ((long long)ph * g.in_w + pw) * g.x_pitch;
      p.o_sw = (long long)st * g.x_pitch; p.o_sh = (long long)st * g.in_w * g.x_pitch;
      p.o_sn = (long long)g.in_h * g.in_w * g.x_pitch;
      p.nnz = reinterpret_cast<const uint32_t*>(pk + L.off_nnz);
      p.nnz_tap_stride = L.n_tiles * L.k_tiles; p.nnz_n_stride = 1; p.nnz_k_stride = L.k_tiles;
      TMaps4 amaps;
      const uint32_t abox[4] = {(uint32_t)kBK, (uint32_t)p.bw, (uint32_t)p.bh, (uint32_t)p.bn};
      rc = make_act_map(&amaps.a[0], dy, g.batch, g.out_h, g.out_w, g.cout, g.cout, 1, 0, 0, abox);
      if (rc != RIGL_OK) return rc;
      for (int i = 1; i < 4; ++i) amaps.a[i] = amaps.a[0];
      const int bn_tile = pick_bn(g.cin);
      CUtensorMap bmap;
      const uint64_t bdims[3] = {(uint64_t)L.cout_pad, (uint64_t)g.cin, (uint64_t)g.taps()};
      const uint64_t bstr[2] = {(uint64_t)L.cout_pad * 2, (uint64_t)g.cin * L.cout_pad * 2};
      const uint32_t bbox[3] = {(uint32_t)kBK, (uint32_t)kmajor_b_rows(p, bn_tile), 1};
      rc = make_tmap(&bmap, pk + L.off_dgrad, 3, bdims, bstr, bbox);
      if (rc != RIGL_OK) return rc;
      CUtensorMap omap = bmap;
      p.tma_store = g_tma_store ? 1 : 0;
      if (p.tma_store) {
        rc = make_act_map(&omap, dx, g.batch, g.in_h, g.in_w, g.cin, g.x_pitch, st, ph, pw, abox);
        if (rc != RIGL_OK) return rc;
      }
      rc = dispatch_kmajor(g.cin, amaps, bmap, omap, p, bn_tile, s);
      if (rc != RIGL_OK) return rc;
    }
  return RIGL_OK;
}

template <int BN, int STAGES, int CL>
static int launch_wgrad_cl(const TMaps4& xmaps, const CUtensorMap& dymap, const WgradParams& p, cudaStream_t s) {
  constexpr size_t smem = (size_t)STAGES * (kBM * kBK * 2 + BN * kBK * 2) + 1024 + 256;
  static_assert(smem <= 227 * 1024, "wgrad kernel exceeds the shared memory of an SM");
  static bool configured = false;
  if (!configured) {
    RIGL_CUDA(cudaFuncSetAttribute(k_igemm_wgrad<BN, STAGES, CL>, cudaFuncAttributeMaxDynamicSharedMemorySize, (int)smem));
    configured = true;
  }
  const int groups = ((p.ntaps * p.m_tiles + CL - 1) / CL) * p.n_tiles * p.splits;
  int clusters = g_num_sms / CL;
  if (groups < clusters) clusters = groups;
  const int rc = launch_clustered<CL>(k_igemm_wgrad<BN, STAGES, CL>, clusters * CL, smem, s, xmaps, dymap, p);
  if (rc != RIGL_OK) return rc;
  RIGL_LAUNCH_CHECK("k_igemm_wgrad");
  return RIGL_OK;
}

template <int BN, int STAGES>
static int launch_wgrad(const TMaps4& xmaps, const CUtensorMap& dymap, const WgradParams& p, cudaStream_t s) {
  if constexpr (BN >= 128) {
    if (g_cluster_mc && p.ntaps * p.m_tiles >= 2) return launch_wgrad_cl<BN, STAGES, 2>(xmaps, dymap, p, s);
  }
  return launch_wgrad_cl<BN, STAGES, 1>(xmaps, dymap, p, s);
}

int tc_wgrad(const ConvGeom& g, const void* x, const void* dy, float* dw, float beta, void* ws, size_t ws_bytes,
             cudaStream_t s) {
  int rc = ensure_driver();
  if (rc != RIGL_OK) return rc;
  {
    HaloParams hp = {};
    if (halo_wgrad_ok(g, &hp)) {
      const size_t need = halo_wgrad_ws_elems(g, hp) * sizeof(float);
      float* wsf = reinterpret_cast<float*>((reinterpret_cast<uintptr_t>(ws) + 255) & ~(uintptr_t)255);
      if (ws == nullptr || ws_bytes < need + 256) {
        set_error("rigl_conv2d_wgrad_dense: workspace %zu < required %zu", ws_bytes, need + 256);
        return RIGL_ERR_WORKSPACE;
      }
      rc = halo_launch_wgrad(hp, g, x, dy, wsf, s);
      if (rc != RIGL_OK) return rc;
      const long long n_w9 = (long long)9 * g.cin * g.cout;
      const long long threads = (n_w9 + 3) / 4;
      k_splitk_reduce<<<(unsigned)((threads + 255) / 256), 256, 0, s>>>(wsf, n_w9, halo_wgrad_grid(hp), dw, n_w9, beta);
      RIGL_LAUNCH_CHECK("k_splitk_reduce");
      return RIGL_OK;
    }
  }
  WgradParams p = {};
  set_pixel_tiling(p, g.out_w, g.out_h, g.batch, 64);
  p.pblocks = p.tiles_w * p.tiles_h * p.tiles_n;
  const int bn_tile = wgrad_bn_tile(g);
  const size_t elems = wgrad_ws_elems(g, &p.splits, &p.pblocks_per_split, p.bw, p.bh, p.bn, bn_tile);
  p.ci = g.cin; p.co = g.cout;
  p.m_tiles = (g.cin + kBM - 1) / kBM; p.n_tiles = (g.cout + bn_tile - 1) / bn_tile;
  const long long n_w = (long long)g.taps() * g.cin * g.cout;
  const bool direct = (p.splits == 1 && beta == 0.f);
  if (!direct) {
    const size_t need = elems * sizeof(float);
    if (ws == nullptr || ws_bytes < need + 256) {
      set_error("rigl_conv2d_wgrad_dense: workspace %zu < required %zu", ws_bytes, need + 256);
      return RIGL_ERR_WORKSPACE;
    }
    p.out = reinterpret_cast<float*>((reinterpret_cast<uintptr_t>(ws) + 255) & ~(uintptr_t)255);
    p.split_stride = n_w;
  } else {
    p.out = dw; p.split_stride = 0;
  }
  TMaps4 xmaps;
  const uint32_t box[4] = {64, (uint32_t)p.bw, (uint32_t)p.bh, (uint32_t)p.bn};
  rc = set_conv_taps(p, &xmaps, g, x, box);
  if (rc != RIGL_OK) return rc;
  CUtensorMap dymap;
  rc = make_act_map(&dymap, dy, g.batch, g.out_h, g.out_w, g.cout, g.cout, 1, 0, 0, box);
  if (rc != RIGL_OK) return rc;
  rc = (bn_tile == 128) ? launch_wgrad<128, 6>(xmaps, dymap, p, s) : launch_wgrad<64, 8>(xmaps, dymap, p, s);
  if (rc != RIGL_OK) return rc;
  if (!direct) {
    const long long threads = (n_w + 3) / 4;
    k_splitk_reduce<<<(unsigned)((threads + 255) / 256), 256, 0, s>>>(p.out, p.split_stride, p.splits, dw, n_w, beta);
    RIGL_LAUNCH_CHECK("k_splitk_reduce");
  }
  return RIGL_OK;
}

}
```

rigl_b200/csrc/mask_ops.cu:

```cuda
#include <string.h>

#include "common.cuh"

namespace rigl {

std::atomic<uint64_t> g_launches{0};
static thread_local char g_err[512] = "";

void set_error(const char* fmt, ...) {
  va_list ap;
  va_start(ap, fmt);
  vsnprintf(g_err, sizeof(g_err), fmt, ap);
  va_end(ap);
}

__global__ void k_pack_f32(const float* __restrict__ src, int64_t n, uint32_t* __restrict__ bits,
                           int64_t words) {
  const int64_t word = (int64_t)blockIdx.x * (blockDim.x >> 5) + (threadIdx.x >> 5);
  if (word >= words) return;
  const int lane = threadIdx.x & 31;
  const int64_t e = word * 32 + lane;
  const bool on = e < n && src[e] != 0.0f;
  const uint32_t w = __ballot_sync(0xffffffffu, on);
  if (lane == 0) bits[word] = w;
}

__global__ void k_unpack_f32(const uint32_t* __restrict__ bits, int64_t n, float* __restrict__ dst) {
  const int64_t e = (int64_t)blockIdx.x * blockDim.x + threadIdx.x;
  if (e < n) dst[e] = ((bits[e >> 5] >> (e & 31)) & 1u) ? 1.0f : 0.0f;
}

__global__ void k_popcount(const uint32_t* __restrict__ bits, int64_t words, int32_t* out) {
  uint32_t c = 0;
  for (int64_t i = (int64_t)blockIdx.x * blockDim.x + threadIdx.x; i < words;
       i += (int64_t)gridDim.x * blockDim.x)
    c += __popc(bits[i]);
#pragma unroll
  for (int o = 16; o > 0; o >>= 1) c += __shfl_xor_sync(0xffffffffu, c, o);
  if ((threadIdx.x & 31) == 0 && c) atomicAdd(out, (int32_t)c);
}

__global__ void k_apply_mask_f32(const float* __restrict__ src, const uint32_t* __restrict__ bits,
                                 int64_t n, float* __restrict__ dst, float scale) {
  const int64_t t = (int64_t)blockIdx.x * blockDim.x + threadIdx.x;
  const int64_t e0 = t * 4;
  if (e0 >= n) return;
  const uint32_t nib = (bits[e0 >> 5] >> (e0 & 31)) & 0xFu;
  if (e0 + 3 < n) {
    float4 v = *reinterpret_cast<const float4*>(src + e0);
    v.x = (nib & 1u) ? v.x * scale : 0.f;
    v.y = (nib & 2u) ? v.y * scale : 0.f;
    v.z = (nib & 4u) ? v.z * scale : 0.f;
    v.w = (nib & 8u) ? v.w * scale : 0.f;
    *reinterpret_cast<float4*>(dst + e0) = v;
  } else {
    for (int c = 0; c < 4 && e0 + c < n; ++c) dst[e0 + c] = ((nib >> c) & 1u) ? src[e0 + c] * scale : 0.f;
  }
}

}

using namespace rigl;

extern "C" int rigl_version(void) { return 203; }
extern "C" const char* rigl_last_error(void) { return g_err; }
extern "C" uint64_t rigl_launch_count(void) { return g_launches.load(); }

extern "C" int rigl_mask_pack_f32(const float* src, int64_t n, uint32_t* bits, void* stream) {
  RIGL_REQUIRE(src && bits && n > 0, "rigl_mask_pack_f32: bad arguments");
  const int64_t words = rigl_mask_words(n);
  const int wpb = 8;
  k_pack_f32<<<(unsigned)((words + wpb - 1) / wpb), wpb * 32, 0, (cudaStream_t)stream>>>(src, n, bits, words);
  RIGL_LAUNCH_CHECK("k_pack_f32");
  return RIGL_OK;
}

extern "C" int rigl_mask_unpack_f32(const uint32_t* bits, int64_t n, float* dst, void* stream) {
  RIGL_REQUIRE(dst && bits && n > 0, "rigl_mask_unpack_f32: bad arguments");
  k_unpack_f32<<<(unsigned)((n + 255) / 256), 256, 0, (cudaStream_t)stream>>>(bits, n, dst);
  RIGL_LAUNCH_CHECK("k_unpack_f32");
  return RIGL_OK;
}

extern "C" int rigl_mask_popcount(const uint32_t* bits, int64_t n, int32_t* out_count_dev, void* stream) {
  RIGL_REQUIRE(bits && out_count_dev && n > 0, "rigl_mask_popcount: bad arguments");
  const int64_t words = rigl_mask_words(n);
  RIGL_CUDA(cudaMemsetAsync(out_count_dev, 0, sizeof(int32_t), (cudaStream_t)stream));
  int blocks = (int)((words + 255) / 256);
  if (blocks > kNumSmsHint * 4) blocks = kNumSmsHint * 4;
  k_popcount<<<blocks, 256, 0, (cudaStream_t)stream>>>(bits, words, out_count_dev);
  RIGL_LAUNCH_CHECK("k_popcount");
  return RIGL_OK;
}

extern "C" int rigl_apply_mask_f32(const float* src, const uint32_t* bits, int64_t n, float* dst,
                                   float scale, void* stream) {
  RIGL_REQUIRE(src && bits && dst && n > 0, "rigl_apply_mask_f32: bad arguments");
  RIGL_REQUIRE(aligned16(src) && aligned16(dst), "rigl_apply_mask_f32: src/dst must be 16-byte aligned");
  const int64_t threads = (n + 3) / 4;
  k_apply_mask_f32<<<(unsigned)((threads + 255) / 256), 256, 0, (cudaStream_t)stream>>>(src, bits, n, dst, scale);
  RIGL_LAUNCH_CHECK("k_apply_mask_f32");
  return RIGL_OK;
}
```

rigl_b200/layers.py:

```python
import math

import numpy as np
import torch
from torch import nn

from . import _cabi
from . import pruning
from .masks import MaskVariable

import ctypes as C

_WS = {}
import os as _os
FUSE_BN_STATS = _os.environ.get('RIGL_FUSE_BN_STATS', '1') != '0'
FUSE_BN_INFER = _os.environ.get('RIGL_FUSE_BN_INFER', '1') != '0'
_BN_ROWS = []


def _bn_partial_rows():
  if not _BN_ROWS:
    _BN_ROWS.append(int(_cabi.lib().rigl_bn_partial_rows()))
  return _BN_ROWS[0]


STEM_S2D_PATH = _os.environ.get('RIGL_STEM_S2D', '1') != '0'


class Profiler(object):
  enabled = False
  records = []

  @classmethod
  def start(cls):
    cls.enabled, cls.records = True, []

  @classmethod
  def stop(cls):
    cls.enabled = False
    torch.cuda.synchronize()
    out = [(k, sc, s.elapsed_time(e)) for k, sc, s, e in cls.records]
    cls.records = []
    return out


def _timed(kind, layer, fn):
  if not Profiler.enabled:
    return fn()
  s, e = torch.cuda.Event(enable_timing=True), torch.cuda.Event(enable_timing=True)
  s.record()
  r = fn()
  e.record()
  Profiler.records.append((kind, layer.scope, s, e))
  return r


def _workspace(device, nbytes):
  key = (device, _WS_SLOT[0])
  ws = _WS.get(key)
  if ws is None or ws.numel() < nbytes:
    ws = torch.empty(max(int(nbytes), 1 << 20), dtype=torch.uint8, device=device)
    _WS[key] = ws
  return ws


WGRAD_SIDE_STREAM = False
MASKED_GRAD_IN_OPTIMIZER = False
DP_HOOK = None
_WS_SLOT = ['main']
_SIDE = {}
_SIDE_KEEP = []


def side_stream(device):
  st = _SIDE.get(device)
  if st is None:
    st = torch.cuda.Stream(device=device)
    _SIDE[device] = st
  return st


_PACKED_AHEAD = set()
_FROZEN = set()


class PackPlan(object):

  def __init__(self):
    self._plan, self._key = C.c_void_p(None), None

  def __del__(self):
    try:
      self._destroy()
    except Exception:
      pass

  def _destroy(self):
    if self._plan and self._plan.value:
      _cabi.lib().rigl_pack_plan_destroy(self._plan)
      self._plan = C.c_void_p(None)

  @staticmethod
  def _entries(layer):
    if getattr(layer, 'patch_mode', False):
      return [(layer.weight.data_ptr(), layer.mask.bits.data_ptr(), layer.packed_patch.data_ptr(), 1, layer._kdim,
               layer._cout)]
    return [(layer.weight.data_ptr(), layer.mask.bits.data_ptr(), layer.packed.data_ptr(), layer._taps, layer._cin,
             layer._cout)]

  def run(self, layers):
    ents = [e for l in layers for e in self._entries(l)]
    key = tuple(ents)
    if key != self._key:
      self._destroy()
      descs = (_cabi.PackDesc * len(ents))()
      for d, (w, b, pk, taps, cin, cout) in zip(descs, ents):
        d.weights, d.mask_bits, d.packed, d.taps, d.cin, d.cout = w, b, pk, taps, cin, cout
      plan = C.c_void_p(None)
      _cabi.check(_cabi.lib().rigl_pack_plan_create(descs, len(ents), C.byref(plan)), 'rigl_pack_plan_create')
      self._plan, self._key = plan, key
    _cabi.check(_cabi.lib().rigl_pack_plan_run(self._plan, _cabi.stream_ptr()), 'rigl_pack_plan_run')
    for l in layers:
      if getattr(l, 's2d_mode', False):
        l.pack_special()


_PACK_PLANS = {}


class _AllLayers(object):
  scope = 'all_layers'


_ALL_LAYERS = _AllLayers()


def pack_all(layers):
  layers = [l for l in layers if l.weight.is_cuda]
  if not layers:
    return
  key = tuple(id(l) for l in layers)
  plan = _PACK_PLANS.get(key)
  if plan is None:
    plan = _PACK_PLANS[key] = PackPlan()
  _timed('pack', _ALL_LAYERS, lambda: plan.run(layers))
  for l in layers:
    _PACKED_AHEAD.add(id(l))


class frozen_operands(object):

  def __init__(self, layers):
    self.ids = set(id(l) for l in layers)

  def __enter__(self):
    self.added = self.ids - _FROZEN
    _FROZEN.update(self.added)
    return self

  def __exit__(self, *exc):
    _FROZEN.difference_update(self.added)
    return False


def _pack_for_forward(layer):
  if id(layer) in _FROZEN:
    return
  if id(layer) in _PACKED_AHEAD:
    _PACKED_AHEAD.discard(id(layer))
    return
  _timed('pack', layer, layer.pack)


def join_side_streams():
  for dev, st in _SIDE.items():
    torch.cuda.current_stream(dev).wait_stream(st)
  del _SIDE_KEEP[:]


class NamedParameter(nn.Parameter):
  name = None
  initial_value = None


class MaskedWeights(object):

  def __init__(self, scope, numel, device):
    self.name = scope + '/masked_weights:0'
    self.dense_grad = torch.zeros(numel, dtype=torch.float32, device=device)
    self.fresh = False


def variance_scaling_(tensor_hwio, scale=2.0):
  fan_in = int(np.prod(tensor_hwio.shape[:-1]))
  with torch.no_grad():
    tensor_hwio.normal_(0., math.sqrt(scale / max(fan_in, 1)))
  return tensor_hwio


class _MaskedConvFn(torch.autograd.Function):

  @staticmethod
  def forward(ctx, x, weight, bias, layer, out_f32):
    _pack_for_forward(layer)
    y = _timed('fprop', layer, lambda: layer._fprop(x, bias, out_f32))
    ctx.layer = layer
    ctx.save_for_backward(x)
    ctx.has_bias = bias is not None
    return y

  @staticmethod
  def backward(ctx, dy):
    layer = ctx.layer
    x, = ctx.saved_tensors
    dy16 = layer._as_activation(dy, layer.out_channels)
    dx = _timed('dgrad', layer, lambda: layer._dgrad(dy16, x)) if ctx.needs_input_grad[0] else None
    mw = layer.masked_weights
    gw = None
    if WGRAD_SIDE_STREAM and x.is_cuda and not Profiler.enabled:
      want_gw = ctx.needs_input_grad[1] and not MASKED_GRAD_IN_OPTIMIZER
      if want_gw and layer.weight.grad is None:
        layer.weight.grad = torch.zeros_like(layer.weight)
      patch_keep = getattr(layer, '_patch_cache', None)
      main, side = torch.cuda.current_stream(x.device), side_stream(x.device)
      side.wait_stream(main)
      _WS_SLOT[0] = 'side'
      try:
        with torch.cuda.stream(side):
          layer._wgrad(x, dy16, mw.dense_grad, accumulate=mw.fresh)
          if want_gw:
            layer.mask.apply_to(mw.dense_grad, out=layer.weight.grad.view(-1))
      finally:
        _WS_SLOT[0] = 'main'
      _SIDE_KEEP.append((x, dy16, patch_keep))
      mw.fresh = True
      mw.dense_grad.rigl_reduced = False
      if DP_HOOK is not None:
        DP_HOOK.layer_done(layer, side)
    else:
      _timed('wgrad', layer, lambda: layer._wgrad(x, dy16, mw.dense_grad, accumulate=mw.fresh))
      mw.fresh = True
      mw.dense_grad.rigl_reduced = False
      if DP_HOOK is not None:
        DP_HOOK.layer_done(layer, None)
      if ctx.needs_input_grad[1] and not MASKED_GRAD_IN_OPTIMIZER:
        gw = layer.mask.apply_to(mw.dense_grad).view(layer.weight.shape)
    gb = None
    if ctx.has_bias and ctx.needs_input_grad[2]:
      gb = dy.float().reshape(-1, layer.out_channels).sum(0) if dy.dim() == 2 else \
          dy.float().sum(dim=(0, 2, 3))
    return dx, gw, gb, None, None


class _MaskedLayer(nn.Module):
  is_rigl_masked_layer = True

  def _setup(self, scope, shape_hwio, device, registry, kernel_initializer):
    self.scope = scope
    w = torch.empty(shape_hwio, dtype=torch.float32, device=device)
    (kernel_initializer or variance_scaling_)(w)
    self.weight = NamedParameter(w)
    self.weight.name = scope + '/weights:0'
    self.mask = MaskVariable(scope, shape_hwio, device)
    self.masked_weights = MaskedWeights(scope, w.numel(), device)
    taps = int(np.prod(shape_hwio[:-2])) if len(shape_hwio) > 2 else 1
    self._taps, self._cin, self._cout = taps, int(shape_hwio[-2]), int(shape_hwio[-1])
    nbytes = int(_cabi.lib().rigl_packed_weights_bytes(taps, self._cin, self._cout))
    self.packed = torch.zeros(nbytes, dtype=torch.uint8, device=device)
    (registry if registry is not None else pruning.default_registry()).register(self)

  @property
  def in_channels(self):
    return self._cin

  @property
  def out_channels(self):
    return self._cout

  def pack(self):
    _cabi.check(_cabi.lib().rigl_pack_masked_weights(
        self.weight.data_ptr(), self.mask.bits.data_ptr(), self._taps, self._cin, self._cout,
        self.packed.data_ptr(), _cabi.stream_ptr()), 'rigl_pack_masked_weights')

  def extra_repr(self):
    return '%s, hwio=%s' % (self.scope, tuple(self.weight.shape))


class SparseConv2d(_MaskedLayer):

  def __init__(self, in_channels, units, kernel_size, strides=1, padding='SAME', name=None,
               kernel_initializer=None, device='cuda', registry=None):
    super(SparseConv2d, self).__init__()
    k = int(kernel_size[0] if isinstance(kernel_size, (tuple, list)) else kernel_size)
    s = int(strides[0] if isinstance(strides, (tuple, list)) else strides)
    if padding not in ('SAME', 'VALID', 'FIXED'):
      raise ValueError('padding must be SAME, VALID or FIXED')
    self.ksize, self.stride = k, s
    self.padding = padding
    self._setup(name or 'Conv', (k, k, int(in_channels), int(units)), device, registry,
                kernel_initializer)
    self.patch_mode = (int(in_channels) % 8 != 0) and k > 1
    if self.patch_mode:
      self._kdim = k * k * int(in_channels)
      self._kpitch = (self._kdim + 7) // 8 * 8
      nbytes = int(_cabi.lib().rigl_packed_weights_bytes(1, self._kdim, self._cout))
      self.packed_patch = torch.zeros(nbytes, dtype=torch.uint8, device=device)
    self.s2d_mode = bool(STEM_S2D_PATH and self.patch_mode and k == 7 and s == 2 and int(in_channels) <= 3 and
                         int(units) <= 64 and int(units) % 8 == 0 and padding == 'FIXED')
    if self.s2d_mode:
      self.packed_s2d = torch.zeros(16 * int(units) * 32, dtype=torch.uint8, device=device)
    self._use_s2d = False
    self.collect_bn_stats = False
    self.bn_partial = None

  def pack(self):
    if self.patch_mode:
      _cabi.check(_cabi.lib().rigl_pack_masked_weights(
          self.weight.data_ptr(), self.mask.bits.data_ptr(), 1, self._kdim, self._cout,
          self.packed_patch.data_ptr(), _cabi.stream_ptr()), 'rigl_pack_masked_weights')
      self.pack_special()
    else:
      super(SparseConv2d, self).pack()

  def pack_special(self):
    if self.patch_mode:
      if self.s2d_mode:
        d = self._desc(1, 16, 16)
        _cabi.check(_cabi.lib().rigl_stem_s2d_pack_weights(
            d, self.weight.data_ptr(), self.mask.bits.data_ptr(), self.packed_s2d.data_ptr(),
            _cabi.stream_ptr()), 'rigl_stem_s2d_pack_weights')

  @property
  def pad(self):
    return 0 if self.padding == 'VALID' else (self.ksize - 1) // 2

  def out_size(self, size):
    k, s = self.ksize, self.stride
    if self.padding == 'SAME':
      out = (size + s - 1) // s
      return out, max((out - 1) * s + k - size, 0) // 2
    if self.padding == 'FIXED':
      return (size + 2 * ((k - 1) // 2) - k) // s + 1, (k - 1) // 2
    return (size - k) // s + 1, 0

  def _desc(self, n, h, w):
    d = _cabi.ConvDesc()
    d.batch, d.in_h, d.in_w, d.cin = n, h, w, self._cin
    d.out_h, pad_h = self.out_size(h)
    d.out_w, pad_w = self.out_size(w)
    if pad_h != pad_w:
      raise ValueError('unequal vertical/horizontal padding is not supported (%d vs %d)' % (pad_h, pad_w))
    d.cout, d.ksize, d.stride, d.pad = self._cout, self.ksize, self.stride, pad_h
    d.x_pitch = 0
    return d

  def _patch_desc(self, rows):
    d = _cabi.ConvDesc()
    d.batch, d.in_h, d.in_w, d.cin = rows, 1, 1, self._kdim
    d.out_h, d.out_w, d.cout, d.ksize, d.stride, d.pad = 1, 1, self._cout, 1, 1, 0
    d.x_pitch = self._kpitch
    return d

  @staticmethod
  def _as_activation(t, channels):
    if t.dtype != torch.bfloat16:
      t = t.to(torch.bfloat16)
    return t.contiguous(memory_format=torch.channels_last)

  def _patches(self, x):
    n, c, h, w = x.shape
    d = self._desc(n, h, w)
    rows = n * d.out_h * d.out_w
    a = torch.empty((rows, self._kpitch), dtype=torch.bfloat16, device=x.device)
    _cabi.check(_cabi.lib().rigl_im2col_nhwc(d, x.data_ptr(), a.data_ptr(), self._kpitch,
                                             _cabi.stream_ptr()), 'rigl_im2col_nhwc')
    return a

  def _fprop(self, x, bias, out_f32):
    n, c, h, w = x.shape
    d = self._desc(n, h, w)
    y = torch.empty((n, self._cout, d.out_h, d.out_w), dtype=torch.bfloat16, device=x.device,
                    memory_format=torch.channels_last)
    packed, src = self.packed, x
    self._use_s2d = bool(self.s2d_mode and _cabi.lib().rigl_stem_s2d_supported(d))
    if self._use_s2d:
      xs = torch.empty(int(_cabi.lib().rigl_stem_s2d_folded_bytes(d)), dtype=torch.uint8, device=x.device)
      _cabi.check(_cabi.lib().rigl_stem_s2d_fold_input(d, x.data_ptr(), xs.data_ptr(), _cabi.stream_ptr()),
                  'rigl_stem_s2d_fold_input')
      _cabi.check(_cabi.lib().rigl_stem_s2d_fprop(d, xs.data_ptr(), self.packed_s2d.data_ptr(), y.data_ptr(),
                                                  _cabi.stream_ptr()), 'rigl_stem_s2d_fprop')
      self._patch_cache = xs
      return y
    if self.patch_mode:
      self._patch_cache = src = self._patches(x)
      d, packed = self._patch_desc(src.shape[0]), self.packed_patch
    ws = _workspace(x.device, _cabi.lib().rigl_conv_workspace_bytes(d))
    self.bn_partial = None
    if self.collect_bn_stats and self.training and FUSE_BN_STATS:
      rows = C.c_int(0)
      part = torch.empty(_bn_partial_rows() * 2 * self._cout, dtype=torch.float32, device=x.device)
      rc = _cabi.lib().rigl_masked_conv2d_fprop_bnstats(
          d, src.data_ptr(), packed.data_ptr(), y.data_ptr(), part.data_ptr(), C.byref(rows), ws.data_ptr(),
          ws.numel(), _cabi.stream_ptr())
      if rc == 0:
        self.bn_partial = (part, rows.value, y.data_ptr())
        return y
      if rc != -4:
        _cabi.check(rc, 'rigl_masked_conv2d_fprop_bnstats')
    _cabi.check(_cabi.lib().rigl_masked_conv2d_fprop(
        d, src.data_ptr(), packed.data_ptr(), y.data_ptr(), None, None, ws.data_ptr(),
        ws.numel(), _cabi.stream_ptr()), 'rigl_masked_conv2d_fprop')
    return y

  def _dgrad(self, dy, x):
    n, c, h, w = x.shape
    d = self._desc(n, h, w)
    if self.patch_mode:
      super(SparseConv2d, self).pack()
    dx = torch.empty_like(x, memory_format=torch.channels_last)
    ws = _workspace(x.device, _cabi.lib().rigl_conv_workspace_bytes(d))
    _cabi.check(_cabi.lib().rigl_masked_conv2d_dgrad(
        d, dy.data_ptr(), self.packed.data_ptr(), dx.data_ptr(), ws.data_ptr(), ws.numel(),
        _cabi.stream_ptr()), 'rigl_masked_conv2d_dgrad')
    return dx

  def _wgrad(self, x, dy, out, accumulate):
    n, c, h, w = x.shape
    d, src = self._desc(n, h, w), x
    if self._use_s2d and getattr(self, '_patch_cache', None) is not None:
      xs, self._patch_cache = self._patch_cache, None
      ws = _workspace(x.device, _cabi.lib().rigl_stem_s2d_workspace_bytes(d))
      _cabi.check(_cabi.lib().rigl_stem_s2d_wgrad(
          d, xs.data_ptr(), dy.data_ptr(), out.data_ptr(), 1.0 if accumulate else 0.0, ws.data_ptr(),
          ws.numel(), _cabi.stream_ptr()), 'rigl_stem_s2d_wgrad')
      return
    if self.patch_mode:
      src = self._patch_cache if getattr(self, '_patch_cache', None) is not None else self._patches(x)
      self._patch_cache = None
      d = self._patch_desc(src.shape[0])
    ws = _workspace(x.device, _cabi.lib().rigl_conv_workspace_bytes(d))
    _cabi.check(_cabi.lib().rigl_conv2d_wgrad_dense(
        d, src.data_ptr(), dy.data_ptr(), out.data_ptr(), 1.0 if accumulate else 0.0, ws.data_ptr(),
        ws.numel(), _cabi.stream_ptr()), 'rigl_conv2d_wgrad_dense')

  def bn_fusable(self, bn):
    return bool(FUSE_BN_INFER and not self.training and bn.uses_inference_form() and not torch.is_grad_enabled())

  def _fprop_bn(self, x, bn, residual):
    if self.patch_mode:
      return None
    n, c, h, w = x.shape
    d = self._desc(n, h, w)
    scale, shift = bn.inference_coefficients()
    out = torch.empty((n, self._cout, d.out_h, d.out_w), dtype=torch.bfloat16, device=x.device,
                      memory_format=torch.channels_last)
    if residual is not None and residual.shape != out.shape:
      raise ValueError('residual of shape %s for an output of shape %s' % (tuple(residual.shape), tuple(out.shape)))
    ws = _workspace(x.device, _cabi.lib().rigl_conv_workspace_bytes(d))
    rc = _cabi.lib().rigl_masked_conv2d_fprop_bnapply(
        d, x.data_ptr(), self.packed.data_ptr(), None if residual is None else residual.data_ptr(), scale.data_ptr(),
        shift.data_ptr(), int(bn.relu), out.data_ptr(), ws.data_ptr(), ws.numel(), _cabi.stream_ptr())
    if rc == -4:
      return None
    _cabi.check(rc, 'rigl_masked_conv2d_fprop_bnapply')
    return out

  def forward(self, x, bn=None, residual=None):
    if x.dim() != 4:
      raise ValueError('Rank not supported {}'.format(x.dim()))
    if x.shape[1] != self._cin:
      raise ValueError('expected %d input channels, got %d' % (self._cin, x.shape[1]))
    x = self._as_activation(x, self._cin)
    if bn is not None and self.bn_fusable(bn):
      if residual is not None:
        residual = residual.to(torch.bfloat16).contiguous(memory_format=torch.channels_last)
      _pack_for_forward(self)
      out = _timed('fprop', self, lambda: self._fprop_bn(x, bn, residual))
      if out is None:
        out = bn(_timed('fprop', self, lambda: self._fprop(x, None, False)), residual=residual)
      return out
    y = _MaskedConvFn.apply(x, self.weight, None, self, False)
    return y if bn is None else bn(y, residual=residual, producer=self)


class SparseLinear(_MaskedLayer):

  def __init__(self, in_features, units, use_bias=True, name=None, kernel_initializer=None,
               device='cuda', registry=None, out_dtype=torch.bfloat16):
    super(SparseLinear, self).__init__()
    self.ksize, self.stride, self.pad = 1, 1, 0
    self.out_dtype = out_dtype
    self._setup(name or 'Dense', (int(in_features), int(units)), device, registry,
                kernel_initializer)
    if use_bias:
      self.bias = NamedParameter(torch.zeros(int(units), dtype=torch.float32, device=device))
      self.bias.name = self.scope + '/biases:0'
    else:
      self.register_parameter('bias', None)

  def _desc(self, m):
    d = _cabi.ConvDesc()
    d.batch, d.in_h, d.in_w, d.cin = m, 1, 1, self._cin
    d.out_h, d.out_w, d.cout, d.ksize, d.stride, d.pad = 1, 1, self._cout, 1, 1, 0
    d.x_pitch = 0
    return d

  @staticmethod
  def _as_activation(t, channels):
    t = t.reshape(-1, channels)
    if t.dtype != torch.bfloat16:
      t = t.to(torch.bfloat16)
    return t.contiguous()

  def _fprop(self, x, bias, out_f32):
    d = self._desc(x.shape[0])
    ws = _workspace(x.device, _cabi.lib().rigl_conv_workspace_bytes(d))
    y16 = None if out_f32 else torch.empty((x.shape[0], self._cout), dtype=torch.bfloat16, device=x.device)
    y32 = torch.empty((x.shape[0], self._cout), dtype=torch.float32, device=x.device) if out_f32 else None
    _cabi.check(_cabi.lib().rigl_masked_conv2d_fprop(
        d, x.data_ptr(), self.packed.data_ptr(), None if y16 is None else y16.data_ptr(),
        None if y32 is None else y32.data_ptr(), None if bias is None else bias.data_ptr(),
        ws.data_ptr(), ws.numel(), _cabi.stream_ptr()), 'rigl_masked_conv2d_fprop')
    return y32 if out_f32 else y16

  def _dgrad(self, dy, x):
    d = self._desc(x.shape[0])
    dx = torch.empty_like(x)
    ws = _workspace(x.device, _cabi.lib().rigl_conv_workspace_bytes(d))
    _cabi.check(_cabi.lib().rigl_masked_conv2d_dgrad(
        d, dy.data_ptr(), self.packed.data_ptr(), dx.data_ptr(), ws.data_ptr(), ws.numel(),
        _cabi.stream_ptr()), 'rigl_masked_conv2d_dgrad')
    return dx

  def _wgrad(self, x, dy, out, accumulate):
    d = self._desc(x.shape[0])
    ws = _workspace(x.device, _cabi.lib().rigl_conv_workspace_bytes(d))
    _cabi.check(_cabi.lib().rigl_conv2d_wgrad_dense(
        d, x.data_ptr(), dy.data_ptr(), out.data_ptr(), 1.0 if accumulate else 0.0, ws.data_ptr(),
        ws.numel(), _cabi.stream_ptr()), 'rigl_conv2d_wgrad_dense')

  def forward(self, x):
    lead = x.shape[:-1]
    x2 = self._as_activation(x, self._cin)
    y = _MaskedConvFn.apply(x2, self.weight, self.bias, self, self.out_dtype == torch.float32)
    return y.reshape(*lead, self._cout)


_SCOPED = {}


def reset_scopes():
  _SCOPED.clear()


def sparse_conv2d(x, units, kernel_size, activation=None, use_bias=False, kernel_initializer=None,
                  kernel_regularizer=None, bias_initializer=None, biases_regularizer=None,
                  sparsity_technique='baseline', normalizer_fn=None, strides=(1, 1), padding='SAME',
                  data_format='channels_last', name=None):
  if data_format not in ('channels_last', 'channels_first'):
    raise ValueError('Not a valid channel string:', data_format)
  if x.dim() != 4:
    raise ValueError('Rank not supported {}'.format(x.dim()))
  key = ('conv', name)
  layer = _SCOPED.get(key) if name else None
  if layer is None:
    if sparsity_technique == 'threshold':
      layer = SparseConv2d(x.shape[1], units, kernel_size, strides=strides, padding=padding,
                           name=name, kernel_initializer=kernel_initializer, device=x.device)
    elif sparsity_technique == 'baseline':
      k = kernel_size[0] if isinstance(kernel_size, (tuple, list)) else kernel_size
      s = strides[0] if isinstance(strides, (tuple, list)) else strides
      layer = nn.Conv2d(x.shape[1], units, k, stride=s, padding=(k - 1) // 2 if padding != 'VALID' else 0,
                        bias=use_bias, device=x.device, dtype=x.dtype)
    else:
      raise ValueError('Unsupported sparsity technique {}'.format(sparsity_technique))
    if name:
      _SCOPED[key] = layer
  y = layer(x)
  if normalizer_fn is not None:
    y = normalizer_fn(y)
  return activation(y) if activation is not None else y


def sparse_fully_connected(x, units, activation=None, use_bias=True, kernel_initializer=None,
                           kernel_regularizer=None, bias_initializer=None, biases_regularizer=None,
                           sparsity_technique='baseline', name=None):
  key = ('dense', name)
  layer = _SCOPED.get(key) if name else None
  if layer is None:
    if sparsity_technique == 'threshold':
      layer = SparseLinear(x.shape[-1], units, use_bias=use_bias, name=name,
                           kernel_initializer=kernel_initializer, device=x.device)
    elif sparsity_technique == 'baseline':
      layer = nn.Linear(x.shape[-1], units, bias=use_bias, device=x.device, dtype=x.dtype)
    else:
      raise ValueError('Unsupported sparsity technique {}'.format(sparsity_technique))
    if name:
      _SCOPED[key] = layer
  y = layer(x)
  return activation(y) if activation is not None else y
```

rigl_b200/norm.py:

```python
import torch
from torch import nn

from . import _cabi
from .layers import _timed, _workspace


def _p(t):
  return None if t is None else t.data_ptr()


class _BNFn(torch.autograd.Function):

  @staticmethod
  def forward(ctx, y, gamma, beta, residual, mod, partial, fork=False):
    n, c, h, w = y.shape
    rows = n * h * w
    dev = y.device
    out = torch.empty_like(y, memory_format=torch.channels_last)
    save = torch.empty((4, c), dtype=torch.float32, device=dev)
    ws = _workspace(dev, _cabi.lib().rigl_bn_workspace_bytes(rows, c) + 8 * c + 256)
    bits = torch.empty(rows * c // 8, dtype=torch.uint8, device=dev) if (residual is not None and mod.relu) else None

    rmean, rvar = (mod.running_mean, mod.running_var) if mod.training else (None, None)

    def run():
      if partial is not None:
        _cabi.check(_cabi.lib().rigl_bn_forward_train_partials(
            y.data_ptr(), _p(residual), gamma.data_ptr(), beta.data_ptr(), partial[0].data_ptr(), partial[1],
            rows, c, mod.eps, mod.momentum, int(mod.relu), _p(rmean),
            _p(rvar), save[0].data_ptr(), save[1].data_ptr(), save[2].data_ptr(),
            save[3].data_ptr(), out.data_ptr(), _p(bits), _cabi.stream_ptr()), 'rigl_bn_forward_train_partials')
        return
      _cabi.check(_cabi.lib().rigl_bn_forward_train(
          y.data_ptr(), _p(residual), gamma.data_ptr(), beta.data_ptr(), rows, c, mod.eps, mod.momentum,
          int(mod.relu), _p(rmean), _p(rvar), save[0].data_ptr(),
          save[1].data_ptr(), save[2].data_ptr(), save[3].data_ptr(), out.data_ptr(), ws.data_ptr(),
          ws.numel(), _p(bits), _cabi.stream_ptr()), 'rigl_bn_forward_train')
    _timed('bn_fwd', mod, run)
    ctx.mod, ctx.has_res, ctx.fork = mod, residual is not None, bool(fork)
    ctx.save_for_backward(y, bits, save)
    if fork:
      ctx.set_materialize_grads(False)
      return out, out.detach()
    return out

  @staticmethod
  def backward(ctx, da, da_b=None):
    y, bits, save = ctx.saved_tensors
    mod = ctx.mod
    n, c, h, w = y.shape
    rows = n * h * w

    def as_grad(t):
      t = t.contiguous(memory_format=torch.channels_last)
      return t if t.dtype == torch.bfloat16 else t.to(torch.bfloat16)
    if ctx.fork:
      if da is None and da_b is None:
        return None, None, None, None, None, None, None
      if da is None:
        da, da_b = da_b, None
    da = as_grad(da)
    if da_b is not None:
      da_b = as_grad(da_b)
      if not ctx.has_res and mod.relu:
        da, da_b = da + da_b, None
    dy = torch.empty_like(y, memory_format=torch.channels_last)
    g_out, dres = None, None
    if ctx.has_res and (mod.relu or da_b is not None):
      g_out = dres = torch.empty_like(y, memory_format=torch.channels_last)
    elif ctx.has_res:
      dres = da
    elif da_b is not None:
      g_out = torch.empty_like(y, memory_format=torch.channels_last)
    dgb = torch.empty((2, c), dtype=torch.float32, device=y.device)
    ws = _workspace(y.device, _cabi.lib().rigl_bn_workspace_bytes(rows, c) + 8 * c + 256)

    def run():
      _cabi.check(_cabi.lib().rigl_bn_backward(
          da.data_ptr(), _p(da_b), y.data_ptr(), save[0].data_ptr(), save[1].data_ptr(), save[2].data_ptr(),
          save[3].data_ptr(), rows, c, int(mod.relu), dy.data_ptr(), _p(g_out), dgb[0].data_ptr(), dgb[1].data_ptr(),
          ws.data_ptr(), ws.numel(), _p(bits), _cabi.stream_ptr()), 'rigl_bn_backward')
    _timed('bn_bwd', mod, run)
    return dy, dgb[0], dgb[1], dres, None, None, None


class FusedBatchNormReLU(nn.Module):

  def __init__(self, channels, relu=True, init_zero=False, eps=1e-5, decay=0.9, device='cuda', name=None):
    super(FusedBatchNormReLU, self).__init__()
    if channels % 8:
      raise ValueError('FusedBatchNormReLU needs channels % 8 == 0')
    self.channels, self.relu, self.eps, self.momentum = channels, bool(relu), float(eps), 1.0 - float(decay)
    self.scope = name or 'batch_normalization'
    self.weight = nn.Parameter(torch.zeros(channels, device=device) if init_zero
                               else torch.ones(channels, device=device))
    self.bias = nn.Parameter(torch.zeros(channels, device=device))
    self.register_buffer('running_mean', torch.zeros(channels, device=device))
    self.register_buffer('running_var', torch.ones(channels, device=device))
    self.batch_statistics = False
    self.frozen_coefficients = None

  def inference_coefficients(self):
    if self.frozen_coefficients is not None:
      return self.frozen_coefficients
    scale = self.weight.detach() * torch.rsqrt(self.running_var + self.eps)
    shift = self.bias.detach() - self.running_mean * scale
    return scale, shift

  def uses_inference_form(self):
    return not self.training and not self.batch_statistics

  def forward(self, y, residual=None, producer=None, fork=False, applied=False):
    if y.dim() != 4 or y.shape[1] != self.channels:
      raise ValueError('expected [N,%d,H,W]' % self.channels)
    if applied:
      return (y, y) if fork else y
    partial = None
    if producer is not None and getattr(producer, 'bn_partial', None) is not None:
      part, nrows, ptr = producer.bn_partial
      if ptr == y.data_ptr() and y.dtype == torch.bfloat16 and y.is_contiguous(memory_format=torch.channels_last):
        partial = (part, nrows)
      producer.bn_partial = None
    y = y.contiguous(memory_format=torch.channels_last)
    if y.dtype != torch.bfloat16:
      y = y.to(torch.bfloat16)
    if residual is not None:
      residual = residual.to(torch.bfloat16).contiguous(memory_format=torch.channels_last)
    if self.training:
      return _BNFn.apply(y, self.weight, self.bias, residual, self, partial, fork)
    if self.batch_statistics:
      with torch.no_grad():
        out = _BNFn.apply(y, self.weight, self.bias, residual, self, partial, False)
      return (out, out) if fork else out
    scale, shift = self.inference_coefficients()
    out = torch.empty_like(y, memory_format=torch.channels_last)
    n, c, h, w = y.shape
    _cabi.check(_cabi.lib().rigl_bn_apply(y.data_ptr(), _p(residual), scale.data_ptr(), shift.data_ptr(),
                                          n * h * w, c, int(self.relu), out.data_ptr(), _cabi.stream_ptr()),
                'rigl_bn_apply')
    return (out, out) if fork else out


class _MaxPoolFn(torch.autograd.Function):

  @staticmethod
  def forward(ctx, x, ksize, stride):
    n, c, h, w = x.shape
    oh, ow = (h + stride - 1) // stride, (w + stride - 1) // stride
    y = torch.empty((n, c, oh, ow), dtype=torch.bfloat16, device=x.device, memory_format=torch.channels_last)
    arg = torch.empty((n, oh, ow, c), dtype=torch.uint8, device=x.device)
    _cabi.check(_cabi.lib().rigl_maxpool_same_forward(x.data_ptr(), n, h, w, c, ksize, stride, y.data_ptr(),
                                                      arg.data_ptr(), _cabi.stream_ptr()),
                'rigl_maxpool_same_forward')
    ctx.save_for_backward(arg)
    ctx.geom = (n, h, w, c, ksize, stride)
    return y

  @staticmethod
  def backward(ctx, dy):
    arg, = ctx.saved_tensors
    n, h, w, c, ksize, stride = ctx.geom
    dy = dy.to(torch.bfloat16).contiguous(memory_format=torch.channels_last)
    dx = torch.empty((n, c, h, w), dtype=torch.bfloat16, device=dy.device, memory_format=torch.channels_last)
    _cabi.check(_cabi.lib().rigl_maxpool_same_backward(dy.data_ptr(), arg.data_ptr(), n, h, w, c, ksize, stride,
                                                       dx.data_ptr(), _cabi.stream_ptr()),
                'rigl_maxpool_same_backward')
    return dx, None, None


def max_pool_same(x, ksize=3, stride=2):
  x = x.to(torch.bfloat16).contiguous(memory_format=torch.channels_last)
  return _MaxPoolFn.apply(x, int(ksize), int(stride))
```

rigl_b200/workloads.py:

```python
import math

import numpy as np
import torch
from torch import nn
import torch.nn.functional as F

from . import pruning
from . import sparse_utils
from .layers import SparseConv2d, SparseLinear, variance_scaling_
from .norm import FusedBatchNormReLU, max_pool_same
from .sparse_optimizers import SparseRigLOptimizer
from .sparse_optimizers_base import GlobalStep

BATCH_NORM_DECAY = 0.9
BATCH_NORM_EPSILON = 1e-5


class DenseConv2d(nn.Conv2d):

  def forward(self, x):
    return F.conv2d(x, self.weight.to(torch.bfloat16), None, self.stride, self.padding, self.dilation, self.groups)


def _BNReLU(channels, relu=True, init_zero=False, device='cuda'):
  return FusedBatchNormReLU(channels, relu=relu, init_zero=init_zero, eps=BATCH_NORM_EPSILON,
                            decay=BATCH_NORM_DECAY, device=device)


def conv_bn(conv, bn, x, residual=None, fork=False):
  if conv.bn_fusable(bn):
    return bn(conv(x, bn=bn, residual=residual), applied=True, fork=fork)
  return bn(conv(x), residual=residual, producer=conv, fork=fork)


FORK_BLOCK_OUTPUTS = True


class _Bottleneck(nn.Module):

  def __init__(self, cin, filters, strides, use_projection, name, device, registry):
    super(_Bottleneck, self).__init__()
    mk = lambda ci, co, k, s, n: SparseConv2d(ci, co, k, strides=s, padding='FIXED', name='resnet_model/' + n,
                                              device=device, registry=registry)
    self.proj = None
    if use_projection:
      self.proj = mk(cin, 4 * filters, 1, strides, 'bottleneck_projection_%s' % name)
      self.proj_bn = _BNReLU(4 * filters, relu=False, device=device)
    self.conv1 = mk(cin, filters, 1, 1, 'bottleneck_1_%s' % name)
    self.bn1 = _BNReLU(filters, device=device)
    self.conv2 = mk(filters, filters, 3, strides, 'bottleneck_2_%s' % name)
    self.bn2 = _BNReLU(filters, device=device)
    self.conv3 = mk(filters, 4 * filters, 1, 1, 'bottleneck_3_%s' % name)
    for conv in (self.proj, self.conv1, self.conv2, self.conv3):
      if conv is not None:
        conv.collect_bn_stats = True
    self.bn3 = _BNReLU(4 * filters, relu=True, init_zero=True, device=device)

  def forward(self, x, x_skip=None, fork=False):
    if x_skip is None:
      x_skip = x
    shortcut = x_skip if self.proj is None else conv_bn(self.proj, self.proj_bn, x_skip)
    y = conv_bn(self.conv1, self.bn1, x)
    y = conv_bn(self.conv2, self.bn2, y)
    return conv_bn(self.conv3, self.bn3, y, residual=shortcut, fork=fork)


class ResNet50(nn.Module):

  def __init__(self, num_classes=1000, device='cuda', registry=None):
    super(ResNet50, self).__init__()
    self.registry = registry if registry is not None else pruning.MaskedLayerRegistry()
    reg = self.registry
    self.initial_conv = SparseConv2d(3, 64, 7, strides=2, padding='FIXED', name='resnet_model/initial_conv',
                                     device=device, registry=reg)
    self.initial_bn = _BNReLU(64, device=device)
    self.initial_conv.collect_bn_stats = True
    blocks = []
    cin = 64
    for g, (filters, n_blocks, stride) in enumerate(((64, 3, 1), (128, 4, 2), (256, 6, 2), (512, 3, 2)), 1):
      blocks.append(_Bottleneck(cin, filters, stride, True, 'block_group_projection_block_group%d' % g,
                                device, reg))
      cin = 4 * filters
      for b in range(1, n_blocks):
        blocks.append(_Bottleneck(cin, filters, 1, False, 'block_group%d_%d_1' % (g, b), device, reg))
    self.blocks = nn.ModuleList(blocks)
    self.final_dense = SparseLinear(
        2048, num_classes, name='resnet_model/final_dense', device=device, registry=reg,
        out_dtype=torch.float32,
        kernel_initializer=lambda w: w.normal_(0., .01))

  def forward(self, x):
    x = conv_bn(self.initial_conv, self.initial_bn, x)
    x = max_pool_same(x, 3, 2)
    x_skip, last = x, len(self.blocks) - 1
    for i, blk in enumerate(self.blocks):
      if i < last and FORK_BLOCK_OUTPUTS:
        x, x_skip = blk(x, x_skip, fork=True)
      else:
        x = blk(x, x_skip)
        x_skip = x
    x = x.mean(dim=(2, 3))
    return self.final_dense(x)


class WideResNet(nn.Module):

  def __init__(self, depth=22, width=2, num_classes=10, droprate=0.3, device='cuda', registry=None):
    super(WideResNet, self).__init__()
    if (depth - 4) % 6 != 0:
      raise ValueError('Depth of ResNet specified not sufficient.')
    self.registry = registry if registry is not None else pruning.MaskedLayerRegistry()
    reg, n_blocks = self.registry, (depth - 4) // 6
    self.conv_1 = DenseConv2d(3, 16, 3, padding=1, bias=False, device=device)
    self.droprate = droprate
    blocks, cin = [], 16
    for name, size, subsample in (('conv_2', 16 * width, False), ('conv_3', 32 * width, True),
                                  ('conv_4', 64 * width, True)):
      for n in range(n_blocks):
        stride = 2 if (subsample and n == 0) else 1
        blk = nn.Module()
        blk.bn_a = _BNReLU(cin, device=device)
        blk.skip = None
        if cin != size:
          blk.skip = SparseConv2d(cin, size, 1, strides=stride, padding='VALID',
                                  name='resnet_model/skip_%s' % name, device=device, registry=reg)
        blk.conv_a = SparseConv2d(cin, size, 3, strides=stride, padding='SAME',
                                  name='resnet_model/%s_%d_1' % (name, n), device=device, registry=reg)
        blk.bn_b = _BNReLU(size, device=device)
        blk.conv_b = SparseConv2d(size, size, 3, strides=1, padding='SAME',
                                  name='resnet_model/%s_%d_2' % (name, n), device=device, registry=reg)
        blocks.append(blk)
        cin = size
    self.blocks = nn.ModuleList(blocks)
    self.final_bn = _BNReLU(cin, device=device)
    self.logits = SparseLinear(cin, num_classes, name='resnet_model/logits', device=device, registry=reg,
                               out_dtype=torch.float32)

  def forward(self, x):
    net = self.conv_1(x.to(torch.bfloat16).contiguous(memory_format=torch.channels_last))
    for blk in self.blocks:
      skip = net
      net = blk.bn_a(net)
      if blk.skip is not None:
        skip = blk.skip(net)
      net = blk.conv_a(net)
      net = F.dropout(blk.bn_b(net), self.droprate, self.training)
      net = blk.conv_b(net) + skip
    net = self.final_bn(net)
    return self.logits(net.mean(dim=(2, 3)))


class MobileNetV1(nn.Module):

  CFG = ((64, 1), (128, 2), (128, 1), (256, 2), (256, 1), (512, 2), (512, 1), (512, 1), (512, 1), (512, 1),
         (512, 1), (1024, 2), (1024, 1))

  def __init__(self, num_classes=1000, device='cuda', registry=None):
    super(MobileNetV1, self).__init__()
    self.registry = registry if registry is not None else pruning.MaskedLayerRegistry()
    reg = self.registry
    self.initial_conv = DenseConv2d(3, 32, 3, stride=2, padding=1, bias=False, device=device)
    self.initial_bn = _BNReLU(32, device=device)
    blocks, cin = [], 32
    for i, (filters, stride) in enumerate(self.CFG):
      blk = nn.Module()
      blk.depthwise = DepthwiseConv2d(cin, stride=stride, device=device)
      blk.bn_dw = _BNReLU(cin, device=device)
      blk.pointwise = SparseConv2d(cin, filters, 1, strides=1, padding='FIXED',
                                   name='resnet_model/contraction_1x1_%d' % i, device=device, registry=reg)
      blk.bn_pw = _BNReLU(filters, device=device)
      blocks.append(blk)
      cin = filters
    self.blocks = nn.ModuleList(blocks)
    self.final_dense = SparseLinear(cin, num_classes, name='resnet_model/final_dense', device=device,
                                    registry=reg, out_dtype=torch.float32)

  def forward(self, x):
    x = self.initial_bn(self.initial_conv(x.to(torch.bfloat16).contiguous(memory_format=torch.channels_last)))
    for blk in self.blocks:
      x = blk.bn_dw(blk.depthwise(x))
      x = conv_bn(blk.pointwise, blk.bn_pw, x)
    return self.final_dense(x.mean(dim=(2, 3)))


def _make_divisible(v, divisor=8, min_value=None):
  if min_value is None:
    min_value = divisor
  new_v = max(min_value, int(v + divisor / 2) // divisor * divisor)
  if new_v < 0.9 * v:
    new_v += divisor
  return new_v


def _trunc_variance_scaling_(t, fan_in):
  std = math.sqrt(1.0 / max(fan_in, 1)) / .87962566103423978
  with torch.no_grad():
    nn.init.trunc_normal_(t, 0., std, -2. * std, 2. * std)
  return t


def _hwio_init(w):
  return _trunc_variance_scaling_(w, int(np.prod(w.shape[:-1])))


MOBILENET_V2_BLOCKS = ((16, 1), (24, 2), (24, 1), (32, 2), (32, 1), (32, 1), (64, 2), (64, 1), (64, 1), (64, 1),
                       (96, 1), (96, 1), (96, 1), (160, 2), (160, 1), (160, 1), (320, 1))


def mobilenet_v2_plan(width=1.0, expansion_factor=6.0):
  def need8(c, layer):
    if c % 8:
      raise ValueError('MobileNetV2(width=%g, expansion_factor=%g): %s has %d channels, not a multiple of 8'
                       % (width, expansion_factor, layer, c))
    return c
  c0 = need8(_make_divisible(32 * width), 'initial_conv')
  blocks, prev = [], c0
  for b, (filters, stride) in enumerate(MOBILENET_V2_BLOCKS):
    expand = need8(int(expansion_factor * prev), 'expand_1x1_%d' % b) if b else None
    cout = need8(_make_divisible(int(width * filters), divisor=8 if b else 1), 'contraction_1x1_%d' % b)
    blocks.append((b, prev, expand, stride, cout, prev == cout and stride == 1))
    prev = cout
  last = need8(max(1280, _make_divisible(1280 * width, 8)), 'final_1x1_conv')
  return c0, blocks, last


class MobileNetV2(nn.Module):

  def __init__(self, num_classes=1000, width=1.0, expansion_factor=6.0, prune_last_layer=True, device='cuda',
               registry=None):
    super(MobileNetV2, self).__init__()
    c0, plan, last = mobilenet_v2_plan(width, expansion_factor)
    self.registry = registry if registry is not None else pruning.MaskedLayerRegistry()
    reg = self.registry

    def mk(ci, co, n):
      conv = SparseConv2d(ci, co, 1, strides=1, padding='FIXED', name='resnet_model/' + n, device=device,
                          registry=reg, kernel_initializer=_hwio_init)
      conv.collect_bn_stats = True
      return conv
    self.initial_conv = DenseConv2d(3, c0, 3, stride=2, padding=1, bias=False, device=device)
    _trunc_variance_scaling_(self.initial_conv.weight, 27)
    self.initial_bn = _BNReLU(c0, device=device)
    blocks = []
    for b, cin, expand, stride, cout, shortcut in plan:
      blk = nn.Module()
      blk.shortcut = shortcut
      blk.expand = None
      mid = cin
      if expand is not None:
        blk.expand = mk(cin, expand, 'expand_1x1_%d' % b)
        blk.bn_expand = _BNReLU(expand, device=device)
        mid = expand
      blk.depthwise = DepthwiseConv2d(mid, stride=stride, device=device)
      bound = math.sqrt(6.0 / (9 * mid + 9))
      with torch.no_grad():
        blk.depthwise.weight.uniform_(-bound, bound)
      blk.bn_dw = _BNReLU(mid, device=device)
      blk.contraction = mk(mid, cout, 'contraction_1x1_%d' % b)
      blk.bn_contraction = _BNReLU(cout, relu=False, device=device)
      blocks.append(blk)
    self.blocks = nn.ModuleList(blocks)
    self.final_conv = mk(plan[-1][4], last, 'final_1x1_conv')
    self.final_bn = _BNReLU(last, device=device)
    self.prune_last_layer = bool(prune_last_layer)
    if self.prune_last_layer:
      self.final_dense = SparseLinear(last, num_classes, name='resnet_model/final_dense', device=device, registry=reg,
                                      out_dtype=torch.float32, kernel_initializer=_hwio_init)
    else:
      self.final_dense = nn.Linear(last, num_classes, device=device)
      with torch.no_grad():
        _trunc_variance_scaling_(self.final_dense.weight, last)
        self.final_dense.bias.zero_()

  def forward(self, x):
    x = self.initial_bn(self.initial_conv(x.to(torch.bfloat16).contiguous(memory_format=torch.channels_last)))
    x_skip = x
    for i, blk in enumerate(self.blocks):
      h = x
      if blk.expand is not None:
        h = conv_bn(blk.expand, blk.bn_expand, h)
      h = blk.bn_dw(blk.depthwise(h))
      fork = FORK_BLOCK_OUTPUTS and i + 1 < len(self.blocks) and self.blocks[i + 1].shortcut
      y = conv_bn(blk.contraction, blk.bn_contraction, h, residual=x_skip if blk.shortcut else None, fork=fork)
      x, x_skip = y if fork else (y, y)
    x = conv_bn(self.final_conv, self.final_bn, x)
    x = x.mean(dim=(2, 3))
    if not self.prune_last_layer:
      x = x.float()
    return self.final_dense(x)


class MnistFC(nn.Module):

  def __init__(self, hidden=(300, 100), device='cuda', registry=None):
    super(MnistFC, self).__init__()
    self.registry = registry if registry is not None else pruning.MaskedLayerRegistry()
    dims = (784,) + tuple(hidden) + (10,)
    self.layers = nn.ModuleList([
        SparseLinear(dims[i], dims[i + 1], name='layer%d' % (i + 1), device=device,
                     registry=self.registry,
                     out_dtype=torch.float32 if i == len(dims) - 2 else torch.bfloat16)
        for i in range(len(dims) - 1)])

  def forward(self, x):
    for i, l in enumerate(self.layers):
      x = l(x)
      if i + 1 < len(self.layers):
        x = F.relu(x)
    return x


def init_masks(model, method, sparsity, custom_sparsity_map=None, seed=0, erk_power_scale=1.0):
  np.random.seed(seed)
  fn = sparse_utils.get_mask_init_fn(model.registry.get_masks(), method, sparsity,
                                     custom_sparsity_map or {}, erk_power_scale=erk_power_scale)
  return fn()


class TrainHarness(object):

  def __init__(self, model, lr=0.1, momentum=0.9, weight_decay=1e-4, label_smoothing=0.1,
               drop_fraction=0.3, drop_fraction_anneal='cosine', begin_step=0, end_step=25000,
               frequency=100, data_parallel=None, optimizer_cls=SparseRigLOptimizer, lr_schedule=None,
               fused_optimizer=None, inner_optimizer='momentum'):
    import os
    if inner_optimizer not in ('momentum', 'adam'):
      raise ValueError("inner_optimizer must be 'momentum' or 'adam', got %r" % (inner_optimizer,))
    if inner_optimizer == 'adam' and fused_optimizer is not None and not fused_optimizer:
      raise ValueError("inner_optimizer='adam' needs the fused optimizer: there is no non-fused Adam with "
                       "tf.train.AdamOptimizer's arithmetic")
    self.model = model
    self.label_smoothing = label_smoothing
    self.lr_schedule = lr_schedule
    on_cuda = next(model.parameters()).is_cuda
    if fused_optimizer is None:
      fused_optimizer = inner_optimizer == 'adam' or (on_cuda and os.environ.get('RIGL_FUSED_SGD', '1') != '0')
    self.fused = bool(fused_optimizer)
    if inner_optimizer == 'adam':
      from .optim import FusedAdam
      self.inner = FusedAdam(model.parameters(), lr=lr, weight_decay=weight_decay)
    elif self.fused:
      from .optim import FusedMomentumSGD
      self.inner = FusedMomentumSGD(model.parameters(), lr=lr, momentum=momentum, nesterov=True,
                                    weight_decay=weight_decay)
    else:
      self.inner = torch.optim.SGD(model.parameters(), lr=lr, momentum=momentum, nesterov=True,
                                   weight_decay=weight_decay, foreach=True)
    self.opt = optimizer_cls(self.inner, begin_step, end_step, frequency, drop_fraction=drop_fraction,
                             drop_fraction_anneal=drop_fraction_anneal,
                             use_tpu=data_parallel is not None).bind(model.registry)
    self.global_step = GlobalStep(0)
    self.dp = data_parallel
    self._dp_overlap = os.environ.get('RIGL_DP_OVERLAP', '0') == '1'
    self._pack_ahead = on_cuda and os.environ.get('RIGL_PACK_AHEAD', '1') != '0'
    if self.dp is not None:
      self.dp.attach(model)
    if self.fused:
      inv = 1.0 / self.dp.world if self.dp is not None else 1.0
      self.inner.attach_masked_layers(model.registry.layers(), grad_scale=inv, other_grad_scale=inv)
      if self.dp is not None:
        self.dp.masked_grads_in_optimizer = True
        self.dp.other_scale_in_optimizer = True

  def _apply_lr_schedule(self):
    if self.lr_schedule is None:
      return
    lr = float(self.lr_schedule(self.global_step.value))
    if self.fused:
      self.inner.set_lr(lr)
    else:
      if getattr(self, 'graphed', False) and lr != self.inner.param_groups[0]['lr']:
        raise RuntimeError('torch.optim.SGD bakes the learning rate into a captured graph: use the fused optimizer '
                           'with an lr schedule')
      for g in self.inner.param_groups:
        g['lr'] = lr

  def enable_cuda_graph(self, images, labels, warmup=3, overlap_wgrad=None):
    import os
    if overlap_wgrad is None:
      overlap_wgrad = os.environ.get('RIGL_WGRAD_OVERLAP', '1') != '0' 
    self._overlap = bool(overlap_wgrad)
    self._sx, self._sy = images.clone(), labels.clone()
    ok = self._capture(warmup)
    if not ok and self.dp is not None and self._dp_overlap:
      self._dp_overlap = False
      ok = self._capture(warmup)
    return ok

  def release_cuda_graph(self):
    self.graphed = False
    for name in ('_g_fb', '_g_opt', '_sloss'):
      if hasattr(self, name):
        setattr(self, name, None)

  def _capture(self, warmup):
    try:
      side = torch.cuda.Stream()
      side.wait_stream(torch.cuda.current_stream())
      with torch.cuda.stream(side):
        for _ in range(warmup):
          self._forward_backward(self._sx, self._sy, set_to_none=False)
      torch.cuda.current_stream().wait_stream(side)
      torch.cuda.synchronize()
      from . import _cabi
      self._g_fb = torch.cuda.CUDAGraph()
      before = _cabi.launch_count()
      with torch.cuda.graph(self._g_fb, capture_error_mode='thread_local'):
        self._sloss = self._forward_backward(self._sx, self._sy, set_to_none=False)
      self.graph_kernel_launches = _cabi.launch_count() - before
      self.replayed_kernel_launches = 0
      self._g_opt = torch.cuda.CUDAGraph()
      if self.fused:
        self.inner.prepare()
      with torch.cuda.graph(self._g_opt, pool=self._g_fb.pool(), capture_error_mode='thread_local'):
        self.inner.step()
      self.graphed = True
    except Exception as e:
      import warnings
      warnings.warn('CUDA-graph capture failed, running eagerly: %r' % (e,))
      torch.cuda.synchronize()
      self.graphed = False
    return self.graphed

  def _forward_backward(self, images, labels, set_to_none):
    from . import layers
    for mw in self.model.registry.get_masked_weights():
      mw.fresh = False
    self.inner.zero_grad(set_to_none=set_to_none)
    if self._pack_ahead:
      layers.pack_all(self.model.registry.layers())
    logits = self.model(images)
    loss = F.cross_entropy(logits.float(), labels, label_smoothing=self.label_smoothing)
    layers.WGRAD_SIDE_STREAM = bool(getattr(self, '_overlap', False))
    layers.MASKED_GRAD_IN_OPTIMIZER = self.fused
    if self.dp is not None and self._dp_overlap:
      self.dp.begin_backward()
      layers.DP_HOOK = self.dp
    try:
      loss.backward()
    finally:
      layers.WGRAD_SIDE_STREAM = False
      layers.MASKED_GRAD_IN_OPTIMIZER = False
      layers.DP_HOOK = None
      if self.dp is not None and self._dp_overlap:
        side = list(layers._SIDE.values()) if getattr(self, '_overlap', False) else []
        self.dp.finish(self.model, producer_streams=side)
      layers.join_side_streams()
    return loss

  def _graphed_step(self, images, labels):
    self._apply_lr_schedule()
    self._sx.copy_(images, non_blocking=True)
    self._sy.copy_(labels, non_blocking=True)
    self._g_fb.replay()
    self.replayed_kernel_launches += self.graph_kernel_launches
    if self.dp is not None and not self._dp_overlap:
      self.dp.reduce_gradients(self.model)
    self.opt.collect_masked_grads()
    gs = self.global_step
    self.opt._global_step = gs
    def inner_step():
      self._g_opt.replay()
      gs.increment()
    self.opt.cond_mask_update_op(gs, inner_step)
    return self._sloss

  def step(self, images, labels):
    if getattr(self, 'graphed', False):
      return self._graphed_step(images, labels)
    self._apply_lr_schedule()
    loss = self._forward_backward(images, labels, set_to_none=self.dp is None)
    if self.dp is not None and not self._dp_overlap:
      self.dp.reduce_gradients(self.model)
    self.opt.collect_masked_grads()
    self.opt.apply_gradients(None, global_step=self.global_step)
    return loss


class _DepthwiseFn(torch.autograd.Function):

  @staticmethod
  def forward(ctx, x, weight, stride):
    from . import _cabi
    n, c, h, w = x.shape
    oh, ow = (h - 1) // stride + 1, (w - 1) // stride + 1
    y = torch.empty((n, c, oh, ow), dtype=torch.bfloat16, device=x.device, memory_format=torch.channels_last)
    _cabi.check(_cabi.lib().rigl_depthwise3x3_fprop(x.data_ptr(), weight.data_ptr(), n, h, w, c, stride, y.data_ptr(),
                                                    _cabi.stream_ptr()), 'rigl_depthwise3x3_fprop')
    ctx.save_for_backward(x, weight)
    ctx.stride = stride
    return y

  @staticmethod
  def backward(ctx, dy):
    from . import _cabi
    from .layers import _workspace
    x, weight = ctx.saved_tensors
    n, c, h, w = x.shape
    dy = dy.to(torch.bfloat16).contiguous(memory_format=torch.channels_last)
    dx = dw = None
    if ctx.needs_input_grad[0]:
      dx = torch.empty_like(x, memory_format=torch.channels_last)
      _cabi.check(_cabi.lib().rigl_depthwise3x3_dgrad(dy.data_ptr(), weight.data_ptr(), n, h, w, c, ctx.stride,
                                                      dx.data_ptr(), _cabi.stream_ptr()), 'rigl_depthwise3x3_dgrad')
    if ctx.needs_input_grad[1]:
      dw = torch.empty_like(weight)
      ws = _workspace(x.device, _cabi.lib().rigl_depthwise3x3_workspace_bytes(n, h, w, c, ctx.stride))
      _cabi.check(_cabi.lib().rigl_depthwise3x3_wgrad(x.data_ptr(), dy.data_ptr(), n, h, w, c, ctx.stride, dw.data_ptr(),
                                                      0.0, ws.data_ptr(), ws.numel(), _cabi.stream_ptr()),
                  'rigl_depthwise3x3_wgrad')
    return dx, dw, None


class DepthwiseConv2d(nn.Module):

  def __init__(self, channels, stride=1, device='cuda'):
    super(DepthwiseConv2d, self).__init__()
    import math
    import os
    self.channels, self.stride = int(channels), int(stride)
    self.weight = nn.Parameter(torch.empty(channels, 1, 3, 3, device=device))
    nn.init.kaiming_uniform_(self.weight, a=math.sqrt(5))
    self.native = os.environ.get('RIGL_NATIVE_DEPTHWISE', '0') == '1'

  def forward(self, x):
    if self.native and x.is_cuda and self.channels % 8 == 0:
      x = x.to(torch.bfloat16).contiguous(memory_format=torch.channels_last)
      return _DepthwiseFn.apply(x, self.weight, self.stride)
    return F.conv2d(x, self.weight.to(torch.bfloat16), None, self.stride, 1, 1, self.channels)
```

Before: 6661.

## Fuse residual gradient and ReLU mask into conv1 dgrad epilogue

Adds a K-major tensor-core dgrad kernel variant whose epilogue TMA-loads the residual-branch gradient, adds it to the dgrad accumulator, and applies the saved ReLU bitmask before storing. This produces the block-output gradient g directly. The Python side links each non-projection block's conv1 to the previous block's bn3, so the BN backward can skip its separate residual-add/ReLU pass. The cost is extra shared memory for the residual slabs, per-element bit loads in the epilogue, and fragile pointer-matching state between autograd nodes, with a fallback to plain dgrad when shapes or pointers don't match.

```diff
diff --git a/include/rigl_b200.h b/include/rigl_b200.h
--- a/include/rigl_b200.h
+++ b/include/rigl_b200.h
@@ -143,6 +143,9 @@
                                               void* y_bf16, void* ws, size_t ws_bytes, void* stream);
 RIGL_API int rigl_masked_conv2d_dgrad(const rigl_conv_desc* d, const void* dy, const void* packed,
                                       void* dx, void* ws, size_t ws_bytes, void* stream);
+RIGL_API int rigl_masked_conv2d_dgrad_residual_g(const rigl_conv_desc* d, const void* dy, const void* packed,
+                                                 void* g_out, const void* da2, const void* relu_bits, void* ws,
+                                                 size_t ws_bytes, void* stream);
 RIGL_API int rigl_conv2d_wgrad_dense(const rigl_conv_desc* d, const void* x, const void* dy,
                                      float* dw, float beta, void* ws, size_t ws_bytes, void* stream);
 RIGL_API int rigl_im2col_nhwc(const rigl_conv_desc* d, const void* x, void* out, int64_t out_pitch,
diff --git a/rigl_b200/_cabi.py b/rigl_b200/_cabi.py
--- a/rigl_b200/_cabi.py
+++ b/rigl_b200/_cabi.py
@@ -79,6 +79,7 @@
     'rigl_masked_conv2d_fprop_bnapply': (C.c_int, [C.POINTER(ConvDesc), _vp, _vp, _vp, _vp, _vp, _i32, _vp, _vp, _sz,
                                                    _vp]),
     'rigl_masked_conv2d_dgrad': (C.c_int, [C.POINTER(ConvDesc), _vp, _vp, _vp, _vp, _sz, _vp]),
+    'rigl_masked_conv2d_dgrad_residual_g': (C.c_int, [C.POINTER(ConvDesc), _vp, _vp, _vp, _vp, _vp, _vp, _sz, _vp]),
     'rigl_conv2d_wgrad_dense': (C.c_int, [C.POINTER(ConvDesc), _vp, _vp, _vp, _f32, _vp, _sz, _vp]),
     'rigl_im2col_nhwc': (C.c_int, [C.POINTER(ConvDesc), _vp, _vp, _i64, _vp]),
     'rigl_stem_s2d_supported': (C.c_int, [C.POINTER(ConvDesc)]),
diff --git a/rigl_b200/csrc/conv_api.cu b/rigl_b200/csrc/conv_api.cu
--- a/rigl_b200/csrc/conv_api.cu
+++ b/rigl_b200/csrc/conv_api.cu
@@ -171,6 +171,22 @@
   return simt_dgrad(g, dy, static_cast<const uint8_t*>(packed) + L.off_fprop, dx, (cudaStream_t)stream);
 }
 
+extern "C" int rigl_masked_conv2d_dgrad_residual_g(const rigl_conv_desc* d, const void* dy, const void* packed,
+                                                  void* g_out, const void* da2, const void* relu_bits, void* ws,
+                                                  size_t ws_bytes, void* stream) {
+  ConvGeom g;
+  int rc = geom_from_desc(d, &g);
+  if (rc != RIGL_OK) return rc;
+  RIGL_REQUIRE(dy && packed && g_out && da2 && relu_bits, "rigl_masked_conv2d_dgrad_residual_g: null argument");
+  RIGL_REQUIRE(g.cin % 8 == 0, "rigl_masked_conv2d_dgrad_residual_g: cin %d is not a multiple of 8", g.cin);
+  RIGL_REQUIRE(aligned16(g_out) && aligned16(da2), "rigl_masked_conv2d_dgrad_residual_g: tensors must be 16-byte aligned");
+  if (force_simt() || !tc_supported(g, 1)) {
+    set_error("rigl_masked_conv2d_dgrad_residual_g: shape not on the K-major tensor-core kernel");
+    return RIGL_ERR_UNSUPPORTED;
+  }
+  return tc_dgrad(g, dy, packed, g_out, ws, ws_bytes, (cudaStream_t)stream, da2, relu_bits);
+}
+
 extern "C" int rigl_conv2d_wgrad_dense(const rigl_conv_desc* d, const void* x, const void* dy, float* dw,
                                        float beta, void* ws, size_t ws_bytes, void* stream) {
   ConvGeom g;
diff --git a/rigl_b200/csrc/conv_common.cuh b/rigl_b200/csrc/conv_common.cuh
--- a/rigl_b200/csrc/conv_common.cuh
+++ b/rigl_b200/csrc/conv_common.cuh
@@ -61,7 +61,7 @@
 int tc_max_ctas();
 void tc_set_bn_stats_always(bool on);
 int tc_dgrad(const ConvGeom& g, const void* dy, const void* packed, void* dx, void* ws,
-             size_t ws_bytes, cudaStream_t s);
+             size_t ws_bytes, cudaStream_t s, const void* da2 = nullptr, const void* relu_bits = nullptr);
 int tc_wgrad(const ConvGeom& g, const void* x, const void* dy, float* dw, float beta, void* ws,
              size_t ws_bytes, cudaStream_t s);
 
diff --git a/rigl_b200/csrc/igemm_tc.cu b/rigl_b200/csrc/igemm_tc.cu
--- a/rigl_b200/csrc/igemm_tc.cu
+++ b/rigl_b200/csrc/igemm_tc.cu
@@ -163,6 +163,30 @@
   }
 }
 
+template <int S, int R>
+__device__ __forceinline__ void stage_slab_g(const float (&d)[R], uint32_t slab, uint32_t d2slab, int row, bool ok0,
+                                             bool ok1, int lane, const uint32_t (&bits)[2][8]) {
+  const uint32_t sh = 2u * (uint32_t)(lane & 3);
+#pragma unroll
+  for (int jj = 0; jj < 8; ++jj) {
+#pragma unroll
+    for (int h = 0; h < 2; ++h) {
+      const int r = row + 8 * h;
+      const int e = 4 * (8 * S + jj) + 2 * h;
+      const uint32_t off = (uint32_t)r * 128u + (uint32_t)((jj ^ (r & 7)) << 4) + (uint32_t)(lane & 3) * 4u;
+      const float2 f = __bfloat1622float2(__floats2bfloat162_rn(d[e], d[e + 1]));
+      uint32_t rw;
+      asm volatile("ld.shared.b32 %0, [%1];" : "=r"(rw) : "r"(d2slab + off) : "memory");
+      __nv_bfloat162 v = __floats2bfloat162_rn(f.x + __uint_as_float(rw << 16), f.y + __uint_as_float(rw & 0xffff0000u));
+      uint32_t w = *reinterpret_cast<uint32_t*>(&v);
+      const uint32_t m = bits[h][jj] >> sh;
+      w &= ((m & 1u) ? 0x0000ffffu : 0u) | ((m & 2u) ? 0xffff0000u : 0u);
+      if (!(h ? ok1 : ok0)) w = 0u;
+      asm volatile("st.shared.b32 [%0], %1;" ::"r"(slab + off), "r"(w) : "memory");
+    }
+  }
+}
+
 template <int R>
 __device__ __forceinline__ void zero_acc(float (&d)[R]) {
 #pragma unroll
@@ -179,17 +203,21 @@
   }
 }
 
-template <int BN, int STAGES, int CL, bool kBnApply>
+template <int BN, int STAGES, int CL, bool kBnApply, bool kFork = false>
 __device__ __forceinline__ void kmajor_body(const TMaps4& amaps, const CUtensorMap& bmap, const CUtensorMap& omap,
-                                            const IgemmParams& p, const CUtensorMap* rmap, const BnEpilogue& ep) {
+                                            const IgemmParams& p, const CUtensorMap* rmap, const BnEpilogue& ep,
+                                            const uint8_t* __restrict__ relu_bits = nullptr) {
+  static_assert(!(kBnApply && kFork), "one epilogue variant at a time");
   extern __shared__ __align__(1024) uint8_t smem_raw[];
   constexpr uint32_t kABytes = kBM * kBK * 2;
   constexpr uint32_t kBBytes = BN * kBK * 2;
   constexpr uint32_t kStageBytes = kABytes + kBBytes;
   constexpr uint32_t kSlabBytes = kBM * 64 * 2;
+  constexpr int kD2Slabs = kFork ? (BN + 63) / 64 : 0;
   const uint32_t smem_base = (smem_u32(smem_raw) + 1023u) & ~1023u;
   const uint32_t out_base = smem_base + STAGES * kStageBytes;
-  const uint32_t bar_base = out_base + 2 * kSlabBytes;
+  const uint32_t d2_base = out_base + 2 * kSlabBytes;
+  const uint32_t bar_base = d2_base + kD2Slabs * kSlabBytes;
   auto full_bar = [&](int s) { return bar_base + 8u * s; };
   auto empty_bar = [&](int s) { return bar_base + 8u * (STAGES + s); };
   const uint32_t res_bar = bar_base + 8u * (2 * STAGES);
@@ -204,6 +232,10 @@
     if constexpr (kBnApply) {
       mbar_init(res_bar, 1);
       if (ep.residual) prefetch_tmap(rmap);
+    }
+    if constexpr (kFork) {
+      mbar_init(res_bar, 1);
+      prefetch_tmap(rmap);
     }
     fence_barrier_init();
   }
@@ -267,6 +299,16 @@
     for (int tile = cluster_id; tile < total; tile += n_clusters, ++tile_ctr) {
       const int n_tile = tile % p.n_tiles;
       const int m_tile = (tile / p.n_tiles) * CL + (int)cta_rank;
+      if constexpr (kFork) {
+        if (issuer) {
+          const int nsl = min(kD2Slabs, (p.N - n_tile * BN + 63) / 64);
+          mbar_arrive_expect_tx(res_bar, (uint32_t)nsl * kSlabBytes);
+          for (int s = 0; s < nsl; ++s)
+            tma_load_4d(d2_base + (uint32_t)s * kSlabBytes, rmap, res_bar, n_tile * BN + 64 * s,
+                        (m_tile % p.tiles_w) * p.bw, ((m_tile / p.tiles_w) % p.tiles_h) * p.bh,
+                        (m_tile / (p.tiles_w * p.tiles_h)) * p.bn);
+        }
+      }
       uint32_t* live = live_cons[wg][tile_ctr & 1];
       if ((cw & 3) == 0) build_live_mask<kBN64>(p, n_tile, lane, live);
       named_bar_sync(3 + wg, 128);
@@ -308,15 +350,32 @@
         ok[h] = pw < p.GW && ph < p.GH && pn < p.NB;
         o_pix[h] = p.o_off + pn * p.o_sn + ph * p.o_sh + pw * p.o_sw;
       }
-      if (kBnApply || p.tma_store) {
+      if (kBnApply || kFork || p.tma_store) {
 #pragma unroll
         for (int s = 0; s < kBN64; ++s) {
           const int co0 = n_tile * BN + 64 * s;
           if (co0 >= p.N) break;
           const uint32_t slab = out_base + (uint32_t)(slab_ctr & 1) * kSlabBytes;
+          uint32_t bits[2][8];
+          if constexpr (kFork) {
+#pragma unroll
+            for (int h = 0; h < 2; ++h)
+#pragma unroll
+              for (int jj = 0; jj < 8; ++jj)
+                bits[h][jj] = (ok[h] && co0 + 8 * jj < p.N) ? __ldg(relu_bits + ((o_pix[h] + co0 + 8 * jj) >> 3)) : 0u;
+          }
           if (issuer) tma_store_wait_read<1>();
           named_bar_sync(1, kConsumerThreads);
-          if constexpr (kBnApply) {
+          if constexpr (kFork) {
+            if (s == 0) {
+              mbar_wait(res_bar, res_phase);
+              res_phase ^= 1u;
+              stage_slab_g<0>(acc, slab, d2_base, row, ok[0], ok[1], lane, bits);
+            } else {
+              stage_slab_g<(kBN64 > 1 ? 1 : 0)>(acc, slab, d2_base + (uint32_t)s * kSlabBytes, row, ok[0], ok[1], lane,
+                                                bits);
+            }
+          } else if constexpr (kBnApply) {
             if (ep.residual) {
               if (issuer) {
                 mbar_arrive_expect_tx(res_bar, kSlabBytes);
@@ -340,6 +399,7 @@
           if (bn_row && wg == 0) slab_bn_stats(slab, cw, lane, bn_row, co0, p.N);
           ++slab_ctr;
         }
+        if constexpr (kFork) named_bar_sync(1, kConsumerThreads);
       } else {
 #pragma unroll
         for (int jc = 0; jc < BN / 8; ++jc) {
@@ -377,6 +437,14 @@
                   const __grid_constant__ CUtensorMap omap, const IgemmParams p,
                   const __grid_constant__ CUtensorMap rmap, const BnEpilogue ep) {
   kmajor_body<BN, STAGES, CL, true>(amaps, bmap, omap, p, &rmap, ep);
+}
+
+template <int BN, int STAGES, int CL>
+__global__ void __launch_bounds__(kThreads, 1)
+k_igemm_kmajor_fork(const __grid_constant__ TMaps4 amaps, const __grid_constant__ CUtensorMap bmap,
+                    const __grid_constant__ CUtensorMap omap, const IgemmParams p,
+                    const __grid_constant__ CUtensorMap d2map, const uint8_t* __restrict__ relu_bits) {
+  kmajor_body<BN, STAGES, CL, false, true>(amaps, bmap, omap, p, &d2map, BnEpilogue{}, relu_bits);
 }
 
 struct WgradParams {
@@ -744,10 +812,25 @@
 
 template <int BN, int STAGES, int CL>
 static int launch_kmajor(const TMaps4& amaps, const CUtensorMap& bmap, const CUtensorMap& omap, const IgemmParams& p,
-                         cudaStream_t s, const CUtensorMap* rmap, const BnEpilogue* ep) {
+                         cudaStream_t s, const CUtensorMap* rmap, const BnEpilogue* ep, const uint8_t* relu_bits) {
   constexpr size_t smem = (size_t)STAGES * (kBM * kBK * 2 + BN * kBK * 2) + 2 * (kBM * 64 * 2) + 1024 + 256;
   static_assert(smem <= 227 * 1024, "K-major kernel exceeds the shared memory of an SM");
   static_assert(8 * (2 * STAGES + 1) <= 256, "K-major kernel barriers exceed their shared memory");
+  if (relu_bits != nullptr) {
+    constexpr size_t smem_fork = smem + (size_t)((BN + 63) / 64) * (kBM * 64 * 2);
+    static_assert(smem_fork <= 227 * 1024, "K-major residual-g kernel exceeds the shared memory of an SM");
+    static bool configured_fork = false;
+    if (!configured_fork) {
+      RIGL_CUDA(cudaFuncSetAttribute(k_igemm_kmajor_fork<BN, STAGES, CL>,
+                                     cudaFuncAttributeMaxDynamicSharedMemorySize, (int)smem_fork));
+      configured_fork = true;
+    }
+    const int rc = launch_clustered<CL>(k_igemm_kmajor_fork<BN, STAGES, CL>, kmajor_grid(p), smem_fork, s, amaps,
+                                        bmap, omap, p, *rmap, relu_bits);
+    if (rc != RIGL_OK) return rc;
+    RIGL_LAUNCH_CHECK("k_igemm_kmajor_fork");
+    return RIGL_OK;
+  }
   if (ep != nullptr) {
     static bool configured_bn = false;
     if (!configured_bn) {
@@ -774,14 +857,14 @@
 
 static int dispatch_kmajor(int n_out, const TMaps4& amaps, const CUtensorMap& bmap, const CUtensorMap& omap,
                            IgemmParams& p, int bn_tile, cudaStream_t s, const CUtensorMap* rmap = nullptr,
-                           const BnEpilogue* ep = nullptr) {
+                           const BnEpilogue* ep = nullptr, const uint8_t* relu_bits = nullptr) {
   p.n_tiles = (n_out + bn_tile - 1) / bn_tile;
   const bool mc = kmajor_use_mc(p);
   if (bn_tile == 64)
-    return mc ? launch_kmajor<64, 7, 2>(amaps, bmap, omap, p, s, rmap, ep)
-              : launch_kmajor<64, 7, 1>(amaps, bmap, omap, p, s, rmap, ep);
-  return mc ? launch_kmajor<128, 5, 2>(amaps, bmap, omap, p, s, rmap, ep)
-            : launch_kmajor<128, 5, 1>(amaps, bmap, omap, p, s, rmap, ep);
+    return mc ? launch_kmajor<64, 7, 2>(amaps, bmap, omap, p, s, rmap, ep, relu_bits)
+              : launch_kmajor<64, 7, 1>(amaps, bmap, omap, p, s, rmap, ep, relu_bits);
+  return mc ? launch_kmajor<128, 5, 2>(amaps, bmap, omap, p, s, rmap, ep, relu_bits)
+            : launch_kmajor<128, 5, 1>(amaps, bmap, omap, p, s, rmap, ep, relu_bits);
 }
 
 static int pick_bn(int n_out) {
@@ -870,7 +953,7 @@
 }
 
 int tc_dgrad(const ConvGeom& g, const void* dy, const void* packed, void* dx, void* ws, size_t ws_bytes,
-             cudaStream_t s) {
+             cudaStream_t s, const void* da2, const void* relu_bits) {
   (void)ws; (void)ws_bytes;
   int rc = ensure_driver();
   if (rc != RIGL_OK) return rc;
@@ -879,7 +962,12 @@
   const int st = g.stride;
   {
     HaloParams hp = {};
-    if (halo_dgrad_ok(g, &hp))
+    const bool halo = halo_dgrad_ok(g, &hp);
+    if (da2 != nullptr && (halo || st != 1 || !g_tma_store || g.x_pitch != g.cin)) {
+      set_error("residual-g dgrad: not on the stride-1 K-major TMA-store kernel");
+      return RIGL_ERR_UNSUPPORTED;
+    }
+    if (halo)
       return halo_launch_kmajor(hp, dy, g.cout, g.cout, pk + L.off_dgrad, L.cout_pad, g.cin, dx, g.x_pitch, true, s);
   }
   bool need_zero = false;
@@ -933,6 +1021,13 @@
         rc = make_act_map(&omap, dx, g.batch, g.in_h, g.in_w, g.cin, g.x_pitch, st, ph, pw, abox);
         if (rc != RIGL_OK) return rc;
       }
+      if (da2 != nullptr) {
+        CUtensorMap d2map;
+        rc = make_act_map(&d2map, da2, g.batch, g.in_h, g.in_w, g.cin, g.cin, 1, 0, 0, abox);
+        if (rc != RIGL_OK) return rc;
+        return dispatch_kmajor(g.cin, amaps, bmap, omap, p, bn_tile, s, &d2map, nullptr,
+                               static_cast<const uint8_t*>(relu_bits));
+      }
       rc = dispatch_kmajor(g.cin, amaps, bmap, omap, p, bn_tile, s);
       if (rc != RIGL_OK) return rc;
     }
diff --git a/rigl_b200/csrc/mask_ops.cu b/rigl_b200/csrc/mask_ops.cu
--- a/rigl_b200/csrc/mask_ops.cu
+++ b/rigl_b200/csrc/mask_ops.cu
@@ -62,7 +62,7 @@
 
 using namespace rigl;
 
-extern "C" int rigl_version(void) { return 203; }
+extern "C" int rigl_version(void) { return 204; }
 extern "C" const char* rigl_last_error(void) { return g_err; }
 extern "C" uint64_t rigl_launch_count(void) { return g_launches.load(); }
 
diff --git a/rigl_b200/layers.py b/rigl_b200/layers.py
--- a/rigl_b200/layers.py
+++ b/rigl_b200/layers.py
@@ -14,6 +14,7 @@
 import os as _os
 FUSE_BN_STATS = _os.environ.get('RIGL_FUSE_BN_STATS', '1') != '0'
 FUSE_BN_INFER = _os.environ.get('RIGL_FUSE_BN_INFER', '1') != '0'
+FUSE_BN_BWD = _os.environ.get('RIGL_BN_BWD_EPILOGUE', '1') != '0'
 _BN_ROWS = []
 
 
@@ -206,6 +207,13 @@
     ctx.layer = layer
     ctx.save_for_backward(x)
     ctx.has_bias = bias is not None
+    ctx.bn_link = None
+    bn_ref = getattr(layer, 'input_bn', None)
+    bn = bn_ref() if bn_ref is not None else None
+    if bn is not None and FUSE_BN_BWD:
+      link, bn.bwd_link = bn.bwd_link, None
+      if link is not None and link[0] == x.data_ptr() and tuple(link[1]) == tuple(x.shape):
+        ctx.bn_link = (bn, link[0], link[2])
     return y
 
   @staticmethod
@@ -213,7 +221,10 @@
     layer = ctx.layer
     x, = ctx.saved_tensors
     dy16 = layer._as_activation(dy, layer.out_channels)
-    dx = _timed('dgrad', layer, lambda: layer._dgrad(dy16, x)) if ctx.needs_input_grad[0] else None
+    dx = None
+    if ctx.needs_input_grad[0]:
+      link, ctx.bn_link = ctx.bn_link, None
+      dx = _timed('dgrad', layer, lambda: layer._dgrad(dy16, x) if link is None else layer._dgrad_g(dy16, x, link))
     mw = layer.masked_weights
     gw = None
     if WGRAD_SIDE_STREAM and x.is_cuda and not Profiler.enabled:
@@ -311,6 +322,7 @@
     self._use_s2d = False
     self.collect_bn_stats = False
     self.bn_partial = None
+    self.input_bn = None
 
   def pack(self):
     if self.patch_mode:
@@ -422,6 +434,24 @@
         d, dy.data_ptr(), self.packed.data_ptr(), dx.data_ptr(), ws.data_ptr(), ws.numel(),
         _cabi.stream_ptr()), 'rigl_masked_conv2d_dgrad')
     return dx
+
+  def _dgrad_g(self, dy, x, link):
+    bn, ptr, bits = link
+    pend, bn.pending_da2 = bn.pending_da2, None
+    if pend is None or pend[1] != ptr:
+      return self._dgrad(dy, x)
+    n, c, h, w = x.shape
+    d = self._desc(n, h, w)
+    g = torch.empty_like(x, memory_format=torch.channels_last)
+    ws = _workspace(x.device, _cabi.lib().rigl_conv_workspace_bytes(d))
+    rc = _cabi.lib().rigl_masked_conv2d_dgrad_residual_g(
+        d, dy.data_ptr(), self.packed.data_ptr(), g.data_ptr(), pend[0].data_ptr(), bits.data_ptr(), ws.data_ptr(),
+        ws.numel(), _cabi.stream_ptr())
+    if rc == -4:
+      return self._dgrad(dy, x)
+    _cabi.check(rc, 'rigl_masked_conv2d_dgrad_residual_g')
+    bn.pending_g = g.data_ptr()
+    return g
 
   def _wgrad(self, x, dy, out, accumulate):
     n, c, h, w = x.shape
diff --git a/rigl_b200/norm.py b/rigl_b200/norm.py
--- a/rigl_b200/norm.py
+++ b/rigl_b200/norm.py
@@ -2,11 +2,17 @@
 from torch import nn
 
 from . import _cabi
+from . import layers
 from .layers import _timed, _workspace
 
 
 def _p(t):
   return None if t is None else t.data_ptr()
+
+
+def _as_grad(t):
+  t = t.contiguous(memory_format=torch.channels_last)
+  return t if t.dtype == torch.bfloat16 else t.to(torch.bfloat16)
 
 
 class _BNFn(torch.autograd.Function):
@@ -38,7 +44,11 @@
           ws.numel(), _p(bits), _cabi.stream_ptr()), 'rigl_bn_forward_train')
     _timed('bn_fwd', mod, run)
     ctx.mod, ctx.has_res, ctx.fork = mod, residual is not None, bool(fork)
+    ctx.res_ptr = _p(residual)
     ctx.save_for_backward(y, bits, save)
+    mod.bwd_link = None
+    if layers.FUSE_BN_BWD and mod.output_conv_linked and residual is not None and fork and mod.relu:
+      mod.bwd_link = (out.data_ptr(), tuple(out.shape), bits)
     if fork:
       ctx.set_materialize_grads(False)
       return out, out.detach()
@@ -46,27 +56,38 @@
 
   @staticmethod
   def backward(ctx, da, da_b=None):
-    y, bits, save = ctx.saved_tensors
     mod = ctx.mod
-    n, c, h, w = y.shape
-    rows = n * h * w
-
-    def as_grad(t):
-      t = t.contiguous(memory_format=torch.channels_last)
-      return t if t.dtype == torch.bfloat16 else t.to(torch.bfloat16)
+    pend_g, mod.pending_g = mod.pending_g, None
     if ctx.fork:
       if da is None and da_b is None:
         return None, None, None, None, None, None, None
       if da is None:
         da, da_b = da_b, None
-    da = as_grad(da)
+    da = _as_grad(da)
+    g_ready = pend_g is not None and pend_g == da.data_ptr()
+    if pend_g is not None and not g_ready:
+      raise RuntimeError('%s: the dgrad epilogue stored g, but the backward received another gradient' % mod.scope)
+    dy, dgb, dres = _BNFn._backward(ctx, da, None if g_ready else da_b, g_ready)
+    sb = mod.shortcut_bn() if (ctx.has_res and mod.shortcut_bn is not None and layers.FUSE_BN_BWD) else None
+    if sb is not None:
+      sb.pending_da2 = (dres, ctx.res_ptr)
+    return dy, dgb[0], dgb[1], dres, None, None, None
+
+  @staticmethod
+  def _backward(ctx, da, da_b, g_ready):
+    y, bits, save = ctx.saved_tensors
+    mod = ctx.mod
+    n, c, h, w = y.shape
+    rows = n * h * w
     if da_b is not None:
-      da_b = as_grad(da_b)
+      da_b = _as_grad(da_b)
       if not ctx.has_res and mod.relu:
         da, da_b = da + da_b, None
     dy = torch.empty_like(y, memory_format=torch.channels_last)
     g_out, dres = None, None
-    if ctx.has_res and (mod.relu or da_b is not None):
+    if g_ready:
+      dres = da
+    elif ctx.has_res and (mod.relu or da_b is not None):
       g_out = dres = torch.empty_like(y, memory_format=torch.channels_last)
     elif ctx.has_res:
       dres = da
@@ -78,10 +99,11 @@
     def run():
       _cabi.check(_cabi.lib().rigl_bn_backward(
           da.data_ptr(), _p(da_b), y.data_ptr(), save[0].data_ptr(), save[1].data_ptr(), save[2].data_ptr(),
-          save[3].data_ptr(), rows, c, int(mod.relu), dy.data_ptr(), _p(g_out), dgb[0].data_ptr(), dgb[1].data_ptr(),
-          ws.data_ptr(), ws.numel(), _p(bits), _cabi.stream_ptr()), 'rigl_bn_backward')
+          save[3].data_ptr(), rows, c, 0 if g_ready else int(mod.relu), dy.data_ptr(), _p(g_out), dgb[0].data_ptr(),
+          dgb[1].data_ptr(), ws.data_ptr(), ws.numel(), None if g_ready else _p(bits), _cabi.stream_ptr()),
+          'rigl_bn_backward')
     _timed('bn_bwd', mod, run)
-    return dy, dgb[0], dgb[1], dres, None, None, None
+    return dy, dgb, dres
 
 
 class FusedBatchNormReLU(nn.Module):
@@ -99,6 +121,11 @@
     self.register_buffer('running_var', torch.ones(channels, device=device))
     self.batch_statistics = False
     self.frozen_coefficients = None
+    self.output_conv_linked = False
+    self.shortcut_bn = None
+    self.bwd_link = None
+    self.pending_g = None
+    self.pending_da2 = None
 
   def inference_coefficients(self):
     if self.frozen_coefficients is not None:
diff --git a/rigl_b200/workloads.py b/rigl_b200/workloads.py
--- a/rigl_b200/workloads.py
+++ b/rigl_b200/workloads.py
@@ -1,4 +1,5 @@
 import math
+import weakref
 
 import numpy as np
 import torch
@@ -34,6 +35,11 @@
 
 
 FORK_BLOCK_OUTPUTS = True
+
+
+def link_bn_to_conv(bn, conv):
+  conv.input_bn = weakref.ref(bn)
+  bn.output_conv_linked = True
 
 
 class _Bottleneck(nn.Module):
@@ -83,6 +89,10 @@
       cin = 4 * filters
       for b in range(1, n_blocks):
         blocks.append(_Bottleneck(cin, filters, 1, False, 'block_group%d_%d_1' % (g, b), device, reg))
+    for prev, blk in zip(blocks, blocks[1:]):
+      if blk.proj is None:
+        link_bn_to_conv(prev.bn3, blk.conv1)
+        blk.bn3.shortcut_bn = weakref.ref(prev.bn3)
     self.blocks = nn.ModuleList(blocks)
     self.final_dense = SparseLinear(
         2048, num_classes, name='resnet_model/final_dense', device=device, registry=reg,
```

Result: no change. 6683 (median of 6 runs) (+0.3%).
